# theblackcat102/edgedict

Hardware: AMD Instinct MI355X
Metric: utterances/sec (E6D2, 15 s audio) (higher is better)
Workload: dtype bf16; 1 GPU; E6D2 full training step (dither+log-mel+stack3+SpecAugment masks -> 6x1024 LSTM encoder, 2x time reduction -> 2x256 LSTM prediction net -> joint 640 -> RNN-T loss -> backward -> grad all-reduce -> Adam); 64 x 15 s utterances per GPU, U=64, V=2048, ragged lengths; lattice [64,201,65,2048]; global_batch=64, parallelism=dp1

## Files before the change

edgedict_amd/csrc/encoder_stack.hip:

```cpp
#include <stdio.h>
#include <stdlib.h>

#include <algorithm>
#include <mutex>
#include <vector>

#include "stack_kernels.hpp"

int ed_gemm_quiet_partials(int dtype_in, const void* A, long long lda, int a_kmajor, const void* B,
                           long long ldb, int b_kmajor, int M, int N, int K, int split_k,
                           int max_wg_per_cu, float* partials, int* slices, hipStream_t stream);

namespace {

__device__ __forceinline__ uint4 pack8(const float* v) {
    uint4 o;
    o.x = (unsigned)f32_to_bf16(v[0]) | ((unsigned)f32_to_bf16(v[1]) << 16);
    o.y = (unsigned)f32_to_bf16(v[2]) | ((unsigned)f32_to_bf16(v[3]) << 16);
    o.z = (unsigned)f32_to_bf16(v[4]) | ((unsigned)f32_to_bf16(v[5]) << 16);
    o.w = (unsigned)f32_to_bf16(v[6]) | ((unsigned)f32_to_bf16(v[7]) << 16);
    return o;
}
__device__ __forceinline__ int row_of_kap(int kap, int H) { return ((kap >> 4) & 3) * H + (kap >> 6) * 16 + (kap & 15); }

__global__ void pack_wih_kernel(const float* __restrict__ W, const float* __restrict__ b_ih,
                                const float* __restrict__ b_hh, bf16_t* __restrict__ Wp,
                                bf16_t* __restrict__ Wt, float* __restrict__ bp, int H, int I) {
    const long long n = 4ll * H * I;
    for (long long i = (long long)blockIdx.x * blockDim.x + threadIdx.x; i < n;
         i += (long long)gridDim.x * blockDim.x) {
        const int row = (int)(i / I), k = (int)(i % I);
        const int g = row / H, j = row % H;
        const int kap = ed_gate_col(g, j);
        const bf16_t v = f32_to_bf16(W[i]);
        Wp[(long long)kap * I + k] = v;
        if (Wt) Wt[(long long)k * 4 * H + kap] = v;
        if (k == 0) bp[kap] = b_ih[row] + b_hh[row];
    }
}
__global__ void pack_wih8_kernel(const float* __restrict__ W, const float* __restrict__ b_ih,
                                 const float* __restrict__ b_hh, bf16_t* __restrict__ Wp, float* __restrict__ bp, int H,
                                 int I) {
    const int I8 = I >> 3;
    const long long n8 = 4ll * H * I8;
    for (long long c = (long long)blockIdx.x * blockDim.x + threadIdx.x; c < n8; c += (long long)gridDim.x * blockDim.x) {
        const int kap = (int)(c / I8), k8 = (int)(c % I8);
        const int row = row_of_kap(kap, H);
        float v[8];
        const float4 a = *reinterpret_cast<const float4*>(W + (long long)row * I + k8 * 8);
        const float4 b = *reinterpret_cast<const float4*>(W + (long long)row * I + k8 * 8 + 4);
        v[0] = a.x; v[1] = a.y; v[2] = a.z; v[3] = a.w; v[4] = b.x; v[5] = b.y; v[6] = b.z; v[7] = b.w;
        *reinterpret_cast<uint4*>(Wp + (long long)kap * I + k8 * 8) = pack8(v);
        if (k8 == 0) bp[kap] = b_ih[row] + b_hh[row];
    }
}
__global__ __launch_bounds__(256) void pack_wih_t_kernel(const float* __restrict__ W, bf16_t* __restrict__ Wt, int H,
                                                         int I) {
    __shared__ __attribute__((aligned(16))) bf16_t tile[64][64 + 8];
    const int kt = (I + 63) >> 6;
    const int kap0 = (blockIdx.x / kt) * 64, k0 = (blockIdx.x % kt) * 64;
    const int tid = threadIdx.x;
    for (int q = tid; q < 64 * 16; q += 256) {
        const int r = q >> 4, c4 = (q & 15) * 4;
        const int row = row_of_kap(kap0 + r, H);
        float v[4] = {0.f, 0.f, 0.f, 0.f};
        if ((I & 3) == 0 && k0 + c4 + 3 < I) {
            const float4 a = *reinterpret_cast<const float4*>(W + (long long)row * I + k0 + c4);
            v[0] = a.x; v[1] = a.y; v[2] = a.z; v[3] = a.w;
        } else {
            for (int e = 0; e < 4; ++e)
                if (k0 + c4 + e < I) v[e] = W[(long long)row * I + k0 + c4 + e];
        }
        for (int e = 0; e < 4; ++e) tile[c4 + e][r] = f32_to_bf16(v[e]);
    }
    __syncthreads();
    for (int q = tid; q < 64 * 8; q += 256) {
        const int k = q >> 3, c8 = (q & 7) * 8;
        if (k0 + k < I)
            *reinterpret_cast<uint4*>(Wt + (long long)(k0 + k) * 4 * H + kap0 + c8) = *reinterpret_cast<const uint4*>(&tile[k][c8]);
    }
}
__global__ void pack_whh_fwd_kernel(const float* __restrict__ W, bf16_t* __restrict__ out, int H) {
    const long long n8 = 4ll * H * H / 8;
    const int KS = H >> 5;
    for (long long c = (long long)blockIdx.x * blockDim.x + threadIdx.x; c < n8; c += (long long)gridDim.x * blockDim.x) {
        const int lane = (int)(c & 63);
        const long long blk = c >> 6;
        const int g = (int)(blk & 3), ks = (int)((blk >> 2) % KS), ub = (int)((blk >> 2) / KS);
        const int row = g * H + ub * 16 + (lane & 15);
        const int k = ks * 32 + (lane >> 4) * 8;
        float v[8];
        const float4 a = *reinterpret_cast<const float4*>(W + (long long)row * H + k);
        const float4 b = *reinterpret_cast<const float4*>(W + (long long)row * H + k + 4);
        v[0] = a.x; v[1] = a.y; v[2] = a.z; v[3] = a.w; v[4] = b.x; v[5] = b.y; v[6] = b.z; v[7] = b.w;
        *reinterpret_cast<uint4*>(out + c * 8) = pack8(v);
    }
}
__global__ void pack_whh_bwd_kernel(const float* __restrict__ W, bf16_t* __restrict__ out, int H) {
    const long long n8 = 4ll * H * H / 8;
    const int KS = H >> 3;
    for (long long c = (long long)blockIdx.x * blockDim.x + threadIdx.x; c < n8; c += (long long)gridDim.x * blockDim.x) {
        const int lane = (int)(c & 63);
        const long long blk = c >> 6;
        const int n2 = (int)(blk & 1), ks = (int)((blk >> 1) % KS), nb = (int)((blk >> 1) / KS);
        const int unit = (nb * 2 + n2) * 16 + (lane & 15);
        const int kap = ks * 32 + (lane >> 4) * 8;
        const float* src = W + (long long)row_of_kap(kap, H) * H + unit;
        float v[8];
#pragma unroll
        for (int e = 0; e < 8; ++e) v[e] = src[(long long)e * H];
        *reinterpret_cast<uint4*>(out + c * 8) = pack8(v);
    }
}
__global__ void unpermute_rows_kernel(const float* __restrict__ src, long long slice_stride, int S,
                                      float* __restrict__ dst, float* __restrict__ dst2, int H, int K,
                                      int accumulate) {
    const long long n = 4ll * H * K;
    for (long long i = (long long)blockIdx.x * blockDim.x + threadIdx.x; i < n;
         i += (long long)gridDim.x * blockDim.x) {
        const int row = (int)(i / K), k = (int)(i % K);
        const long long o = (long long)ed_gate_col(row / H, row % H) * K + k;
        float v = 0.f;
        for (int sl = 0; sl < S; ++sl) v += src[sl * slice_stride + o];
        dst[i] = accumulate ? dst[i] + v : v;
        if (dst2) dst2[i] = accumulate ? dst2[i] + v : v;
    }
}

__global__ void unpermute_rows4_kernel(const float* __restrict__ src, long long slice_stride, int S,
                                       float* __restrict__ dst, float* __restrict__ dst2, int H, int K,
                                       int accumulate) {
    const int K4 = K >> 2;
    const long long n4 = 4ll * H * K4;
    for (long long c = (long long)blockIdx.x * blockDim.x + threadIdx.x; c < n4; c += (long long)gridDim.x * blockDim.x) {
        const int row = (int)(c / K4), k = (int)(c % K4) * 4;
        const long long o = (long long)ed_gate_col(row / H, row % H) * K + k;
        float4 v = make_float4(0.f, 0.f, 0.f, 0.f);
        for (int sl = 0; sl < S; ++sl) {
            const float4 p = *reinterpret_cast<const float4*>(src + sl * slice_stride + o);
            v.x += p.x; v.y += p.y; v.z += p.z; v.w += p.w;
        }
        const long long i = (long long)row * K + k;
        if (accumulate) {
            const float4 d = *reinterpret_cast<const float4*>(dst + i);
            *reinterpret_cast<float4*>(dst + i) = make_float4(d.x + v.x, d.y + v.y, d.z + v.z, d.w + v.w);
            if (dst2) {
                const float4 e = *reinterpret_cast<const float4*>(dst2 + i);
                *reinterpret_cast<float4*>(dst2 + i) = make_float4(e.x + v.x, e.y + v.y, e.z + v.z, e.w + v.w);
            }
        } else {
            *reinterpret_cast<float4*>(dst + i) = v;
            if (dst2) *reinterpret_cast<float4*>(dst2 + i) = v;
        }
    }
}
int unpermute_rows(const float* src, long long slice_stride, int S, float* dst, float* dst2, int H, int K, int accumulate,
                   hipStream_t s) {
    const bool vec = K % 4 == 0 && slice_stride % 4 == 0 && (uintptr_t)src % 16 == 0 && (uintptr_t)dst % 16 == 0 &&
                     (uintptr_t)dst2 % 16 == 0;
    if (vec)
        hipLaunchKernelGGL(unpermute_rows4_kernel, dim3(ed_grid_for(4ll * H * K / 4, 256, 4096)), dim3(256), 0, s, src,
                           slice_stride, S, dst, dst2, H, K, accumulate);
    else
        hipLaunchKernelGGL(unpermute_rows_kernel, dim3(ed_grid_for(4ll * H * K, 256, 4096)), dim3(256), 0, s, src,
                           slice_stride, S, dst, dst2, H, K, accumulate);
    ED_CHECK_LAUNCH("unpermute_rows_kernel");
    return ED_OK;
}

struct Runtime {
    std::mutex mu;
    hipStream_t R = nullptr, W = nullptr;
    int prio_hi = 0;
    hipEvent_t tev[2][2] = {{nullptr, nullptr}, {nullptr, nullptr}};
    int tlaunches[2] = {0, 0};
    int tkind[2] = {0, 0}, tsteps[2] = {0, 0};
    bool time_each = false;
    static constexpr int STAMP_SLOTS = 4096;
    unsigned long long* stamps[2] = {nullptr, nullptr};
    int stamp_used[2] = {0, 0};
    unsigned long long* stamp_slot(int i, hipStream_t s) {
        if (!time_each) return nullptr;
        if (!stamps[i] && hipMalloc((void**)&stamps[i], (size_t)STAMP_SLOTS * 16) != hipSuccess) {
            stamps[i] = nullptr;
            return nullptr;
        }
        if (stamp_used[i] == 0) {
            if (hipMemsetAsync(stamps[i], 0, (size_t)STAMP_SLOTS * 16, s) != hipSuccess) return nullptr;
            if (hipMemset2DAsync(stamps[i], 16, 0xff, 8, STAMP_SLOTS, s) != hipSuccess) return nullptr;
        }
        if (stamp_used[i] >= STAMP_SLOTS) return nullptr;
        return stamps[i] + 2 * (size_t)stamp_used[i]++;
    }
    unsigned* wsr_err_host = nullptr;
    unsigned* wsr_err_dev = nullptr;
    hipStream_t lazy(hipStream_t& s) {
        if (!s && hipStreamCreateWithPriority(&s, hipStreamNonBlocking, prio_hi) != hipSuccess) s = nullptr;
        return s;
    }
    hipStream_t S[ED_STACK_MAX_SLOTS] = {};
    std::vector<hipEvent_t> pool;
    size_t used = 0;
    hipEvent_t get() {
        if (used == pool.size()) {
            hipEvent_t e;
            if (hipEventCreateWithFlags(&e, hipEventDisableTiming) != hipSuccess) return nullptr;
            pool.push_back(e);
        }
        return pool[used++];
    }
};
std::mutex g_rt_mu;
std::vector<Runtime*> g_rt;

Runtime* runtime_for_current_device() {
    int dev = 0;
    if (hipGetDevice(&dev) != hipSuccess) return nullptr;
    std::lock_guard<std::mutex> registry(g_rt_mu);
    if ((int)g_rt.size() <= dev) g_rt.resize(dev + 1, nullptr);
    if (!g_rt[dev]) {
        Runtime* r = new Runtime();
        int lo = 0, hi = 0;
        if (hipDeviceGetStreamPriorityRange(&lo, &hi) != hipSuccess) lo = hi = 0;
        const char* e = getenv("EDGEDICT_AUX_PRIORITY");
        const bool aux_high = e && e[0] == '1';
        r->prio_hi = hi;
        bool ok = hipStreamCreateWithPriority(&r->R, hipStreamNonBlocking, hi) == hipSuccess &&
                  hipStreamCreateWithPriority(&r->W, hipStreamNonBlocking, aux_high ? hi : lo) == hipSuccess &&
                  hipStreamCreateWithPriority(&r->S[0], hipStreamNonBlocking, hi) == hipSuccess;
        if (!ok) {
            delete r;
            return nullptr;
        }
        for (int i = 0; i < 2; ++i)
            for (int j = 0; j < 2; ++j)
                if (hipEventCreate(&r->tev[i][j]) != hipSuccess) r->tev[i][j] = nullptr;
        if (hipHostMalloc((void**)&r->wsr_err_host, 64, hipHostMallocMapped) == hipSuccess) {
            r->wsr_err_host[0] = r->wsr_err_host[1] = r->wsr_err_host[2] = 0;
            if (hipHostGetDevicePointer((void**)&r->wsr_err_dev, r->wsr_err_host, 0) != hipSuccess)
                r->wsr_err_dev = nullptr;
        }
        g_rt[dev] = r;
    }
    return g_rt[dev];
}

struct Geom {
    int T, f, m, cf, off, nchunks;
};

size_t align256(size_t x) { return (x + 255) / 256 * 256; }
constexpr int LNB_GRID = 128;
constexpr int LNB_GRID_TOP = 512;

struct WsLayout {
    std::vector<size_t> frag0, frag1, dC, lnpart;
    std::vector<size_t> himg;
    size_t himg_stride = 0;
    std::vector<size_t> gimg;
    size_t gimg_stride = 0;
    std::vector<size_t> skpart;
    size_t tmpW = 0, tmpB = 0, dX0 = 0, wsr_sync = 0, total = 0;
};
constexpr size_t SYNC_FFLAG = 0, SYNC_BFLAG = 8 * 512, SYNC_FCNT = 2 * 8 * 512;
constexpr size_t SYNC_BCNT = SYNC_FCNT + (size_t)8 * LPW_CNT_STRIDE;
constexpr size_t SYNC_GCNT = 16 * 1024;
constexpr size_t WSR_SYNC_BYTES = (SYNC_GCNT + (size_t)8 * SK_CNT_LINES * 64) * 4;
static_assert(SYNC_BCNT + (size_t)8 * LPW_CNT_STRIDE <= SYNC_GCNT, "sync region layout");

WsLayout ws_layout(const edgedict_stack_desc_t* d) {
    WsLayout w;
    const size_t B16 = (size_t)(d->B + 15) / 16 * 16;
    size_t off = 0;
    size_t maxK = d->H;
    for (int l = 0; l < d->L; ++l) {
        const size_t fb = align256(B16 * 4 * d->H * sizeof(bf16_t));
        w.frag0.push_back(off); off += fb;
        w.frag1.push_back(off); off += fb;
        if ((size_t)d->layers[l].I > maxK) maxK = d->layers[l].I;
    }
    for (int l = 0; l < d->L; ++l) {
        w.dC.push_back(off);
        off += align256((size_t)d->B * d->H * sizeof(float));
    }
    {
        int f = 1;
        std::vector<int> fl(d->L);
        for (int l = d->L - 1; l >= 0; --l) { f *= max(1, d->layers[l].reduce); fl[l] = f; }
        for (int l = 0; l < d->L; ++l) {
            const int cf = max(1, d->chunk) * fl[l];
            const int nch = (d->layers[l].T + cf - 1) / cf;
            w.lnpart.push_back(off);
            off += align256((size_t)(nch * LNB_GRID + LNB_GRID_TOP) * 2 * d->H * sizeof(float));
        }
    }
    w.tmpW = off; off += align256((size_t)8 * 4 * d->H * maxK * sizeof(float));
    w.tmpB = off; off += align256((size_t)4 * d->H * sizeof(float));
    w.dX0 = off; off += align256((size_t)d->T0 * d->B * d->I0 * sizeof(bf16_t));
    w.wsr_sync = off; off += WSR_SYNC_BYTES;
    w.himg_stride = align256(B16 * d->H * sizeof(bf16_t));
    for (int l = 0; l < d->L; ++l) {
        w.himg.push_back(off);
        off += (size_t)(d->layers[l].T + 1) * w.himg_stride;
    }
    const bool infer = (d->flags & EDGEDICT_STACK_INFERENCE) != 0;
    w.gimg_stride = align256(B16 * 4 * d->H * sizeof(bf16_t));
    for (int l = 0; l < d->L; ++l) {
        w.gimg.push_back(off);
        if (!infer) off += (size_t)(d->layers[l].T + 1) * w.gimg_stride;
    }
    for (int l = 0; l < d->L; ++l) {
        w.skpart.push_back(off);
        if (!infer) off += align256((size_t)2 * (d->H / 64 + 1) * 4 * 64 * 64 * sizeof(float));
    }
    w.total = off;
    return w;
}

int validate(const edgedict_stack_desc_t* d, std::vector<Geom>& g, bool backward) {
    ED_CHECK_ARG(d && d->layers, "encoder_stack: null descriptor");
    ED_CHECK_ARG(d->L >= 1 && d->L <= ED_STACK_MAX_SLOTS, "encoder_stack: 1..%d layers supported (got %d)", ED_STACK_MAX_SLOTS, d->L);
    ED_CHECK_ARG(d->B >= 1 && d->H >= 32 && d->H % 32 == 0 && d->H <= 2048, "encoder_stack: need B >= 1, H %% 32 == 0, H <= 2048 (B=%d H=%d)", d->B, d->H);
    ED_CHECK_ARG(d->chunk >= 1, "encoder_stack: chunk must be >= 1");
    ED_CHECK_ARG(d->T0 >= 1 && d->I0 >= 8 && d->I0 % 8 == 0 && d->I0 <= 1024, "encoder_stack: bad input geometry (T0=%d I0=%d)", d->T0, d->I0);
    ED_CHECK_ARG(d->x && d->in_gamma && d->in_beta && d->in_mean && d->in_rstd && d->out && d->ws, "encoder_stack: null pointer in descriptor");
    g.resize(d->L);
    int f = 1;
    for (int l = d->L - 1; l >= 0; --l) {
        const edgedict_stack_layer_t& y = d->layers[l];
        ED_CHECK_ARG(y.reduce == 1 || y.reduce == 2, "encoder_stack: layer %d: time reduction must be 1 or 2", l);
        f *= y.reduce;
        g[l].f = f;
        g[l].T = y.T;
    }
    int T = d->T0, I = d->I0;
    for (int l = 0; l < d->L; ++l) {
        const edgedict_stack_layer_t& y = d->layers[l];
        ED_CHECK_ARG(y.T == T && y.I == I, "encoder_stack: layer %d geometry (T=%d I=%d) does not follow from the layers above (T=%d I=%d)", l, y.T, y.I, T, I);
        ED_CHECK_ARG(!y.residual || y.I == d->H, "encoder_stack: layer %d: residual needs I == H", l);
        ED_CHECK_ARG(y.drop_p >= 0.f && y.drop_p < 1.f, "encoder_stack: layer %d: dropout probability must be in [0, 1)", l);
        ED_CHECK_ARG(y.wih_p && y.bias_p && y.whh_f && y.ln_gamma && y.ln_beta && y.X && y.G && y.Yx && y.Cx && y.mean && y.rstd, "encoder_stack: layer %d: null pointer", l);
        if (backward)
            ED_CHECK_ARG(y.whh_b && y.dZ && (l == 0 || y.dX) && y.dW_ih && y.dW_hh && y.db && y.dgamma && y.dbeta, "encoder_stack: layer %d: null backward pointer", l);
        g[l].m = g[0].f / g[l].f;
        g[l].cf = d->chunk * g[l].f;
        g[l].nchunks = (y.T + g[l].cf - 1) / g[l].cf;
        T = (T + y.reduce - 1) / y.reduce;
        I = d->H;
    }
    ED_CHECK_ARG(d->ws_bytes >= ws_layout(d).total, "encoder_stack: workspace too small");
    return ED_OK;
}

struct Pace {
    static bool allows(int w, int l, int m_l, int m_min_running) {
        const int period = max(1, m_l / max(1, m_min_running));
        return period <= 1 || ((w + period * 1024 - (l % period)) % period) == 0;
    }
};

int margin_launches(const edgedict_stack_desc_t* d, const std::vector<Geom>& g, bool backward) {
    const int P = d->chunk * g[0].f;
    if (d->lag > 0) return max(1, d->lag - P + (backward ? 1 : 0));
    static const int mf = [] { const char* e = getenv("EDGEDICT_STACK_MARGIN_F"); return e ? atoi(e) : 0; }();
    static const int mb = [] { const char* e = getenv("EDGEDICT_STACK_MARGIN_B"); return e ? atoi(e) : 0; }();
    if (backward ? mb > 0 : mf > 0) return backward ? mb : mf;
    return backward ? 6 : 3;
}

#define ED_TRY(expr)            \
    do {                        \
        int st__ = (expr);      \
        if (st__ != ED_OK) return st__; \
    } while (0)

struct ScheduleTrace {
    int32_t* step_launch = nullptr;
    int32_t* chunk_enqueued = nullptr;
    std::vector<int> toff, coff;
    int launches = 0, max_slots = 0;
};
thread_local ScheduleTrace* g_trace = nullptr;
#define ED_DEV(expr)                      \
    do {                                  \
        if (!g_trace) ED_TRY(expr);       \
    } while (0)

struct Streams {
    hipStream_t C, R, R2, W;
    int split;
    int which(int l) const { return l >= split ? 1 : 0; }
    hipStream_t RS(int l) const { return which(l) ? R2 : R; }
    hipStream_t S[ED_STACK_MAX_SLOTS];
    bool serial;
    Runtime* rt;
    std::unique_lock<std::mutex> lock;
    hipEvent_t shared_ev = nullptr;
    hipStream_t shared_src = nullptr;
    int share(hipStream_t src) {
        if (serial) return ED_OK;
        shared_ev = rt->get();
        ED_CHECK_ARG(shared_ev != nullptr, "encoder_stack: event creation failed");
        ED_CHECK_HIP(hipEventRecord(shared_ev, src));
        shared_src = src;
        return ED_OK;
    }
    void unshare() { shared_ev = nullptr; shared_src = nullptr; }
    int chain(hipStream_t src, hipStream_t waiter) {
        if (serial || src == waiter) return ED_OK;
        if (shared_ev && src == shared_src) {
            ED_CHECK_HIP(hipStreamWaitEvent(waiter, shared_ev, 0));
            return ED_OK;
        }
        hipEvent_t e = rt->get();
        ED_CHECK_ARG(e != nullptr, "encoder_stack: event creation failed");
        ED_CHECK_HIP(hipEventRecord(e, src));
        ED_CHECK_HIP(hipStreamWaitEvent(waiter, e, 0));
        return ED_OK;
    }
    int record(hipEvent_t& e, hipStream_t src) {
        if (serial) return ED_OK;
        e = rt->get();
        ED_CHECK_ARG(e != nullptr, "encoder_stack: event creation failed");
        ED_CHECK_HIP(hipEventRecord(e, src));
        return ED_OK;
    }
    int wait(hipStream_t waiter, hipEvent_t e) {
        if (serial || !e) return ED_OK;
        ED_CHECK_HIP(hipStreamWaitEvent(waiter, e, 0));
        return ED_OK;
    }
};

int open_streams(const edgedict_stack_desc_t* d, void* stream_, Streams& st) {
    st.C = (hipStream_t)stream_;
    st.serial = (d->flags & EDGEDICT_STACK_SERIAL) != 0 || g_trace != nullptr;
    st.rt = nullptr;
    if (st.serial) {
        st.R = st.R2 = st.W = st.C;
        for (auto& x : st.S) x = st.C;
        return ED_OK;
    }
    st.rt = runtime_for_current_device();
    ED_CHECK_ARG(st.rt != nullptr, "encoder_stack: could not create the internal streams");
    st.lock = std::unique_lock<std::mutex>(st.rt->mu);
    st.rt->used = 0;
    st.R = st.rt->R;
    st.R2 = st.rt->R;
    for (int i = 0; i < ED_STACK_MAX_SLOTS; ++i) {
        st.S[i] = st.rt->S[0];
        if ((d->flags & EDGEDICT_STACK_SIDE_STREAM_PER_LAYER) && i > 0) {
// ... 220 lines not shown
            sl.nsteps = t1 - t;
            sl.layer = l;
            ran[Lc.nslot].l = l;
            ran[Lc.nslot].t0 = t;
            ran[Lc.nslot].t1 = t1;
            ++Lc.nslot;
            next_t[l] = t1;
            if (g_trace)
                for (int tt = t; tt < t1; ++tt) g_trace->step_launch[g_trace->toff[l] + tt] = g_trace->launches;
        }
        if (Lc.nslot == 0) {
            ED_CHECK_ARG(++idle < 4096, "encoder_stack: forward schedule made no progress");
            continue;
        }
        idle = 0;
        ++launches;
        Lc.stamp = st.rt ? st.rt->stamp_slot(0, st.R) : nullptr;
        Lc.err = gerr;
        Lc.trace = g_wsr_trace;
        ED_DEV(ed_stack_launch_fwd_lpw(Lc, st.R));
        if (g_trace) {
            g_trace->max_slots = max(g_trace->max_slots, Lc.nslot);
            ++g_trace->launches;
        }
        for (int pass = 0; pass < 2; ++pass) {
            hipStream_t S = pass == 0 ? st.S[0] : st.C;
            EdChunkNorm items[ED_STACK_MAX_SLOTS];
            int idx[ED_STACK_MAX_SLOTS], ni = 0;
            for (int i = 0; i < Lc.nslot; ++i) {
                const int l = ran[i].l;
                if (side(l) != S) continue;
                const edgedict_stack_layer_t& y = d->layers[l];
                EdChunkNorm& e = items[ni];
                e.Yx1 = bptr(y.Yx) + BH;
                e.X = y.residual ? bptr(y.X) : nullptr;
                e.gamma = y.ln_gamma;
                e.beta = y.ln_beta;
                if (l + 1 < L) {
                    e.out = bptr(d->layers[l + 1].X);
                    e.out_st = BH;
                    e.out_sb = H;
                } else {
                    e.out = bptr(d->out);
                    e.out_st = H;
                    e.out_sb = (long long)T_out * H;
                }
                e.mean = y.mean;
                e.rstd = y.rstd;
                e.T = y.T;
                e.t0 = ran[i].t0;
                e.t1 = ran[i].t1;
                e.reduce = y.reduce;
                const DropCfg dc = drop_of(y);
                e.drop_thresh = dc.thresh; e.drop_seed = dc.seed; e.drop_scale = dc.scale; e.drop_T = dc.T_out;
                idx[ni++] = i;
            }
            if (ni == 0) continue;
            if (soft) {
                const unsigned* cp[ED_STACK_MAX_SLOTS];
                unsigned tg[ED_STACK_MAX_SLOTS];
                for (int j = 0; j < ni; ++j) {
                    cp[j] = cnt + (size_t)ran[idx[j]].l * LPW_CNT_STRIDE;
                    tg[j] = (unsigned)WGS * (unsigned)ran[idx[j]].t1;
                }
                ED_DEV(ed_stack_wait_counters(cp, tg, ni, gerr, S));
            } else {
                ED_TRY(st.chain(st.R, S));
            }
            ED_DEV(ed_stack_multi_norm(items, ni, B, H, d->eps, S));
            for (int j = 0; j < ni; ++j) {
                const int i = idx[j];
                const int l = ran[i].l, k = ran[i].t0 / g[l].cf;
                if (l + 1 >= L || ran[i].t1 != min(g[l].T, (k + 1) * g[l].cf)) continue;
                ED_DEV(input_gemm(d, g, l + 1, k, S));
                if (g_trace) g_trace->chunk_enqueued[g_trace->coff[l + 1] + k] = g_trace->launches;
                if (soft) ED_DEV(ed_stack_set_flag(fflag + (l + 1) * 512 + k, S));
                else ED_TRY(st.record(Eg[l + 1][k], S));
                queued[l + 1][k] = 1;
                ready_w[l + 1][k] = w + margin;
            }
            if (st.serial) break;
        }
    }
    if (st.rt && st.rt->tev[0][1]) {
        ED_CHECK_HIP(hipEventRecord(st.rt->tev[0][1], st.R));
        st.rt->tlaunches[0] = launches;
    }
    ED_TRY(st.chain(st.R, st.C));
    for (int l = 0; l < L; ++l) ED_TRY(st.chain(st.S[l], st.C));
    return ED_OK;
}

int lpw_steps(const edgedict_stack_desc_t* d) {
    const char* e_on = getenv("EDGEDICT_STACK_LPW");
    const char* e_n = getenv("EDGEDICT_LPW_STEPS");
    const int on = e_on ? atoi(e_on) : 1, want = e_n ? atoi(e_n) : min(d->chunk, 16);
    if (!on || !ed_stack_lpw_supported(d->B, d->H)) return 0;
    {
        const size_t B16 = (size_t)(d->B + 15) / 16 * 16;
        const size_t stride = align256(B16 * d->H * sizeof(bf16_t));
        for (int l = 0; l < d->L; ++l)
            if ((size_t)(d->layers[l].T + 1) * stride >= (1ull << 32)) return 0;
        if (!g_trace && device_cus() < (d->H >> 4) * ((d->B + 63) >> 6)) return 0;
    }
    bool reduces = false;
    for (int l = 0; l < d->L; ++l) reduces = reduces || d->layers[l].reduce == 2;
    int ns = max(1, min(want, d->chunk));
    while (ns > 1 && (d->chunk % ns != 0 || (reduces && (ns & 1)))) --ns;
    if (reduces && (ns & 1)) return 0;
    return ns;
}

int sk_bwd_steps(const edgedict_stack_desc_t* d) {
    const char* e_on = getenv("EDGEDICT_STACK_BWD_SK");
    const char* e_n = getenv("EDGEDICT_SK_STEPS");
    const int on = e_on ? atoi(e_on) : 1, want = e_n ? atoi(e_n) : min(d->chunk, 16);
    if (!on || !ed_stack_sk_supported(d->B, d->H)) return 0;
    for (int l = 0; l < d->L; ++l)
        if (!d->layers[l].whh_s) return 0;
    {
        const size_t B16 = (size_t)(d->B + 15) / 16 * 16;
        const size_t stride = align256(B16 * 4 * d->H * sizeof(bf16_t));
        for (int l = 0; l < d->L; ++l)
            if ((size_t)(d->layers[l].T + 1) * stride >= (1ull << 32)) return 0;
        if (!g_trace && 2 * device_cus() < (d->H >> 6) * 4) return 0;
    }
    int ns = max(1, min(want, d->chunk));
    while (ns > 1 && d->chunk % ns != 0) --ns;
    return ns;
}

}

extern "C" int edgedict_stack_forward(const edgedict_stack_desc_t* d, void* stream_) {
    std::vector<Geom> g;
    ED_TRY(validate(d, g, false));
    const int B = d->B, H = d->H, L = d->L;
    const long long BH = (long long)B * H;
    const WsLayout wl = ws_layout(d);
    char* ws = (char*)d->ws;
    Streams st;
    ED_TRY(open_streams(d, stream_, st));
    static const int fwd_r2 = [] { const char* e = getenv("EDGEDICT_STACK_FWD_R2"); return e ? atoi(e) : 1; }();
    if (fwd_r2 && !st.serial && st.R2 == st.R) st.R2 = st.C;
    st.split = L;
    if (st.R2 != st.R) {
        st.split = L / 2;
        for (int l = 0; l < L; ++l)
            if (d->layers[l].reduce == 2) { st.split = l + 1; break; }
        if (st.split >= L) st.split = L / 2;
    }

    ED_DEV(ed_stack_input_norm(d->x_dtype, d->x, d->in_gamma, d->in_beta, bptr(d->layers[0].X),
                               d->in_mean, d->in_rstd, B, d->T0, d->I0, d->eps, st.C));
    const int lpw_ns = lpw_steps(d);
    if (lpw_ns && (poison_on() || lpw_data_poll()))
        ED_DEV(ed_stack_fill(ws + wl.himg[0], 0xff,
                             wl.himg[L - 1] + (size_t)(d->layers[L - 1].T + 1) * wl.himg_stride - wl.himg[0], st.C));
    if (st.rt) {
        st.rt->tkind[0] = lpw_ns ? 1 : 0;
        st.rt->tsteps[0] = lpw_ns;
    }
    for (int l0 = 0; l0 < L; l0 += 8) {
        EdInitStates A;
        A.n = min(8, L - l0);
        A.B = B;
        A.H = H;
        for (int j = 0; j < A.n; ++j) {
            const int l = l0 + j;
            const edgedict_stack_layer_t& y = d->layers[l];
            A.h0[j] = d->h0 ? d->h0 + l * BH : nullptr;
            A.c0[j] = d->c0 ? d->c0 + l * BH : nullptr;
            A.Yx0[j] = bptr(y.Yx);
            A.Cx0[j] = y.Cx;
            A.hfrag[j] = bptr(ws + (lpw_ns ? wl.himg[l] : wl.frag0[l]));
        }
        ED_DEV(ed_stack_init_states(A, st.C));
    }
    if (lpw_ns) ED_DEV(ed_stack_zero(ws + wl.wsr_sync, SYNC_BCNT * sizeof(unsigned), st.C));
    ED_TRY(st.chain(st.C, st.R));
    if (st.R2 != st.R) ED_TRY(st.chain(st.C, st.R2));
    for (int l = 0; l < L; ++l) ED_TRY(st.chain(st.C, st.S[l]));

    static const int soft_env = [] { const char* e = getenv("EDGEDICT_STACK_SOFT_WAIT"); return e ? atoi(e) : 1; }();
    const bool soft = soft_env && !st.serial && L <= 8;
    if (lpw_ns) return forward_lpw(d, g, st, wl, lpw_ns, soft);
    unsigned* fflag = reinterpret_cast<unsigned*>(ws + wl.wsr_sync) + SYNC_FFLAG;
    unsigned* gerr = (st.rt && st.rt->wsr_err_dev) ? st.rt->wsr_err_dev + 2 : nullptr;
    if (soft) {
        for (int l = 0; l < L; ++l) ED_CHECK_ARG(g[l].nchunks <= 512, "encoder_stack: too many chunks for the flag table");
        ED_DEV(ed_stack_zero(fflag, (size_t)8 * 512 * sizeof(unsigned), st.C));
        ED_TRY(st.chain(st.C, st.R));
        if (st.R2 != st.R) ED_TRY(st.chain(st.C, st.R2));
        for (int l = 0; l < L; ++l) ED_TRY(st.chain(st.C, st.S[l]));
    }
    std::vector<std::vector<hipEvent_t>> Eg(L);
    std::vector<std::vector<char>> queued(L);
    for (int l = 0; l < L; ++l) {
        Eg[l].assign(g[l].nchunks, nullptr);
        queued[l].assign(g[l].nchunks, 0);
    }
    int next_g0 = 0;
    auto feed_layer0 = [&](int upto) -> int {
        for (; next_g0 < g[0].nchunks && next_g0 <= upto; ++next_g0) {
            ED_DEV(input_gemm(d, g, 0, next_g0, st.S[0]));
            if (g_trace) g_trace->chunk_enqueued[g_trace->coff[0] + next_g0] = g_trace->launches;
            if (soft) ED_DEV(ed_stack_set_flag(fflag + next_g0, st.S[0]));
            else ED_TRY(st.record(Eg[0][next_g0], st.S[0]));
            queued[0][next_g0] = 1;
        }
        return ED_OK;
    };
    ED_TRY(feed_layer0(1));

    const int margin = margin_launches(d, g, false);
    std::vector<int> next_t(L, 0), stepped_w(L, -2);
    std::vector<std::vector<int>> ready_w(L);
    for (int l = 0; l < L; ++l) ready_w[l].assign(g[l].nchunks, l == 0 ? 0 : 0x3fffffff);
    int launches = 0, idle = 0;
    if (st.rt) st.rt->stamp_used[0] = 0;
    if (st.rt && st.rt->tev[0][0]) ED_CHECK_HIP(hipEventRecord(st.rt->tev[0][0], st.R));
    const int T_out = (g[L - 1].T + d->layers[L - 1].reduce - 1) / d->layers[L - 1].reduce;
    struct Done { int l, k; };
    for (int w = 0;; ++w) {
        bool finished = true;
        for (int l = 0; l < L; ++l) finished = finished && next_t[l] >= g[l].T && stepped_w[l] < w - 1;
        if (finished) break;
        EdFwdLaunch Lcs[2];
        for (auto& x : Lcs) {
            x.nstep = x.nnorm = 0;
            x.B = B; x.H = H; x.eps = d->eps;
        }
        Done done[ED_STACK_MAX_SLOTS];
        int ndone = 0;
        for (int l = 0; l < L; ++l) {
            const edgedict_stack_layer_t& y = d->layers[l];
            EdFwdLaunch& Lc = Lcs[st.which(l)];
            if (stepped_w[l] == w - 1) {
                const int t = next_t[l] - 1;
                int ta = -1, tb = -1;
                if (y.reduce == 1) ta = t;
                else if (t & 1) { ta = t - 1; tb = t; }
                else if (t == g[l].T - 1) ta = t;
                if (ta >= 0) {
                    const int tau = ta / y.reduce;
                    EdFwdNorm& n = Lc.norm[Lc.nnorm++];
                    n.y0 = bptr(y.Yx) + (long long)(ta + 1) * BH;
                    n.r0 = y.residual ? bptr(y.X) + (long long)ta * BH : nullptr;
                    n.y1 = tb >= 0 ? bptr(y.Yx) + (long long)(tb + 1) * BH : nullptr;
                    n.r1 = (tb >= 0 && y.residual) ? bptr(y.X) + (long long)tb * BH : nullptr;
                    n.gamma = y.ln_gamma;
                    n.beta = y.ln_beta;
                    if (l + 1 < L) {
                        n.out = bptr(d->layers[l + 1].X) + (long long)tau * BH;
                        n.out_stride = H;
                    } else {
                        n.out = bptr(d->out) + (long long)tau * H;
                        n.out_stride = (long long)T_out * H;
                    }
                    n.mean0 = y.mean + (long long)ta * B;
                    n.rstd0 = y.rstd + (long long)ta * B;
                    n.mean1 = tb >= 0 ? y.mean + (long long)tb * B : nullptr;
                    n.rstd1 = tb >= 0 ? y.rstd + (long long)tb * B : nullptr;
                    n.scale = y.reduce == 1 ? 1.f : 0.5f;
                    const DropCfg dc = drop_of(y);
                    n.drop_thresh = dc.thresh; n.drop_seed = dc.seed; n.drop_scale = dc.scale; n.drop_T = dc.T_out;
                    n.tau = tau;
                }
                const int k = t / g[l].cf;
                if (l + 1 < L && t == min(g[l].T, (k + 1) * g[l].cf) - 1) {
                    done[ndone].l = l;
                    done[ndone].k = k;
                    ++ndone;
                }
            }
            const int t = next_t[l];
            if (t >= g[l].T) continue;
            const int k = t / g[l].cf;
            const bool opens = (t % g[l].cf == 0);
            if (opens && !(queued[l][k] && w >= ready_w[l][k]) && l > 0) continue;
            int m_min = g[l].m;
            for (int j = 0; j < l; ++j)
                if (next_t[j] < g[j].T) m_min = min(m_min, g[j].m);
            if (!Pace::allows(w, l, g[l].m, m_min)) continue;
            if (opens) {
                if (l == 0) ED_TRY(feed_layer0(k + 2));
                ED_CHECK_ARG(queued[l][k], "encoder_stack: schedule violated (layer %d chunk %d)", l, k);
                if (!soft) ED_TRY(st.wait(st.RS(l), Eg[l][k]));
            }
            EdFwdStep& sl = Lc.step[Lc.nstep++];
            sl.wait_flag = (soft && opens) ? fflag + l * 512 + k : nullptr;
            bf16_t* f0 = bptr(ws + wl.frag0[l]);
            bf16_t* f1 = bptr(ws + wl.frag1[l]);
            sl.G_t = bptr(y.G) + (long long)t * B * 4 * H;
            sl.hfrag_in = (t & 1) ? f1 : f0;
            sl.hfrag_out = (t & 1) ? f0 : f1;
            sl.Y_t = bptr(y.Yx) + (long long)(t + 1) * BH;
            sl.C_prev = y.Cx + (long long)t * BH;
            sl.C_t = y.Cx + (long long)(t + 1) * BH;
            sl.Wfrag = bptr(y.whh_f);
            stepped_w[l] = w;
            next_t[l] = t + 1;
            if (g_trace) g_trace->step_launch[g_trace->toff[l] + t] = g_trace->launches;
        }
        if (Lcs[0].nstep + Lcs[0].nnorm + Lcs[1].nstep + Lcs[1].nnorm == 0) {
            ED_CHECK_ARG(++idle < 4096, "encoder_stack: forward schedule made no progress");
            continue;
// ... 21 lines not shown
        }
    }
    const int Wtot = launches;
    if (st.rt && st.rt->tev[0][1]) {
        ED_CHECK_HIP(hipEventRecord(st.rt->tev[0][1], st.R));
        st.rt->tlaunches[0] = Wtot;
    }
    ED_TRY(st.chain(st.R, st.C));
    if (st.R2 != st.R) ED_TRY(st.chain(st.R2, st.C));
    for (int l = 0; l < L; ++l) ED_TRY(st.chain(st.S[l], st.C));
    return ED_OK;
}

extern "C" int edgedict_stack_pack_sk(const float* w_hh, int H, void* whh_s, void* stream_) {
    ED_CHECK_ARG(H >= 64 && H % 64 == 0 && H <= 1024, "stack_pack_sk: needs H %% 64 == 0 and H <= 1024 (got %d)", H);
    ED_CHECK_ARG(w_hh && whh_s, "stack_pack_sk: null pointer");
    return ed_stack_pack_sk(w_hh, (bf16_t*)whh_s, H, (hipStream_t)stream_);
}

extern "C" int edgedict_stack_wsr_set_trace(void* device_buffer) {
    g_wsr_trace = (long long*)device_buffer;
    return ED_OK;
}

extern "C" int edgedict_stack_wsr_error(void) {
    Runtime* r = runtime_for_current_device();
    std::unique_lock<std::mutex> lock;
    if (r) lock = std::unique_lock<std::mutex>(r->mu);
    if (!r || !r->wsr_err_host) return 0;
    volatile unsigned* p = r->wsr_err_host;
    if (!(p[0] | p[1] | p[2])) return 0;
    (void)hipDeviceSynchronize();
    const unsigned code = p[2] ? p[2] : (p[1] ? p[1] : p[0]);
    p[0] = 0;
    p[1] = 0;
    p[2] = 0;
    return (int)code;
}

extern "C" void* edgedict_stack_error_words(int host) {
    Runtime* r = runtime_for_current_device();
    std::unique_lock<std::mutex> lock;
    if (r) lock = std::unique_lock<std::mutex>(r->mu);
    if (!r || !r->wsr_err_host || !r->wsr_err_dev) {
        ed_set_error("stack_error_words: no device runtime");
        return nullptr;
    }
    return host ? (void*)r->wsr_err_host : (void*)r->wsr_err_dev;
}

extern "C" int edgedict_stack_schedule(const edgedict_stack_desc_t* d, int backward, int32_t* step_launch,
                                       int32_t* chunk_enqueued, int32_t* n_launches, int32_t* max_slots) {
    ED_CHECK_ARG(d && step_launch && chunk_enqueued && n_launches && max_slots, "stack_schedule: null pointer");
    ScheduleTrace tr;
    {
        std::vector<Geom> g;
        ED_TRY(validate(d, g, backward != 0));
        int to = 0, co = 0;
        for (int l = 0; l < d->L; ++l) {
            tr.toff.push_back(to);
            tr.coff.push_back(co);
            to += g[l].T;
            co += g[l].nchunks;
        }
        for (int i = 0; i < to; ++i) step_launch[i] = -1;
        for (int i = 0; i < co; ++i) chunk_enqueued[i] = -1;
    }
    tr.step_launch = step_launch;
    tr.chunk_enqueued = chunk_enqueued;
    g_trace = &tr;
    const int rc = backward ? edgedict_stack_backward(d, nullptr) : edgedict_stack_forward(d, nullptr);
    g_trace = nullptr;
    *n_launches = tr.launches;
    *max_slots = tr.max_slots;
    return rc;
}

extern "C" int edgedict_stack_last_timing(int backward, float* ms, int* launches) {
    ED_CHECK_ARG(ms && launches, "stack_last_timing: null pointer");
    Runtime* r = runtime_for_current_device();
    std::unique_lock<std::mutex> lock;
    if (r) lock = std::unique_lock<std::mutex>(r->mu);
    const int i = backward ? 1 : 0;
    ED_CHECK_ARG(r && r->tev[i][0] && r->tev[i][1] && r->tlaunches[i] > 0, "stack_last_timing: nothing recorded");
    ED_CHECK_HIP(hipEventSynchronize(r->tev[i][1]));
    ED_CHECK_HIP(hipEventElapsedTime(ms, r->tev[i][0], r->tev[i][1]));
    *launches = r->tlaunches[i];
    return ED_OK;
}

extern "C" int edgedict_stack_last_mode(int backward, int* kind, int* steps_per_launch) {
    ED_CHECK_ARG(kind && steps_per_launch, "stack_last_mode: null pointer");
    Runtime* r = runtime_for_current_device();
    std::unique_lock<std::mutex> lock;
    if (r) lock = std::unique_lock<std::mutex>(r->mu);
    ED_CHECK_ARG(r, "stack_last_mode: no device runtime");
    *kind = r->tkind[backward ? 1 : 0];
    *steps_per_launch = r->tsteps[backward ? 1 : 0];
    return ED_OK;
}

extern "C" int edgedict_stack_time_launches(int on) {
    Runtime* r = runtime_for_current_device();
    std::unique_lock<std::mutex> lock;
    if (r) lock = std::unique_lock<std::mutex>(r->mu);
    ED_CHECK_ARG(r, "stack_time_launches: no device runtime");
    r->time_each = on != 0;
    return ED_OK;
}

extern "C" int edgedict_stack_launch_times(int backward, float* sum_ms, int* launches) {
    ED_CHECK_ARG(sum_ms && launches, "stack_launch_times: null pointer");
    Runtime* r = runtime_for_current_device();
    std::unique_lock<std::mutex> lock;
    if (r) lock = std::unique_lock<std::mutex>(r->mu);
    const int i = backward ? 1 : 0;
    ED_CHECK_ARG(r && r->stamps[i] && r->stamp_used[i] > 0,
                 "stack_launch_times: nothing recorded (edgedict_stack_time_launches(1) first)");
    const int n = r->stamp_used[i];
    std::vector<unsigned long long> h(2 * (size_t)n);
    ED_CHECK_HIP(hipStreamSynchronize(r->R));
    ED_CHECK_HIP(hipMemcpy(h.data(), r->stamps[i], h.size() * sizeof(unsigned long long), hipMemcpyDeviceToHost));
    double ticks = 0.0;
    int ok = 0;
    for (int k = 0; k < n; ++k)
        if (h[2 * k + 1] > h[2 * k]) {
            ticks += (double)(h[2 * k + 1] - h[2 * k]);
            ++ok;
        }
    ED_CHECK_ARG(ok > 0, "stack_launch_times: no launch stamped");
    *sum_ms = (float)(ticks * 1e-5);
    *launches = ok;
    return ED_OK;
}

extern "C" int edgedict_stack_launch_stamps(int backward, unsigned long long* out, int max_launches, int* launches) {
    ED_CHECK_ARG(out && launches && max_launches > 0, "stack_launch_stamps: bad arguments");
    Runtime* r = runtime_for_current_device();
    std::unique_lock<std::mutex> lock;
    if (r) lock = std::unique_lock<std::mutex>(r->mu);
    const int i = backward ? 1 : 0;
    ED_CHECK_ARG(r && r->stamps[i] && r->stamp_used[i] > 0,
                 "stack_launch_stamps: nothing recorded (edgedict_stack_time_launches(1) first)");
    const int n = min(max_launches, r->stamp_used[i]);
    ED_CHECK_HIP(hipDeviceSynchronize());
    ED_CHECK_HIP(hipMemcpy(out, r->stamps[i], (size_t)n * 16, hipMemcpyDeviceToHost));
    *launches = n;
    return ED_OK;
}

extern "C" int edgedict_stack_backward(const edgedict_stack_desc_t* d, void* stream_) {
    std::vector<Geom> g;
    ED_TRY(validate(d, g, true));
    ED_CHECK_ARG(d->dout && d->d_in_gamma && d->d_in_beta, "encoder_stack: null backward pointer in descriptor");
    ED_CHECK_ARG(!(d->flags & EDGEDICT_STACK_INFERENCE), "encoder_stack: backward on a descriptor flagged EDGEDICT_STACK_INFERENCE");
    const int B = d->B, H = d->H, L = d->L;
    const long long BH = (long long)B * H;
    const WsLayout wl = ws_layout(d);
    char* ws = (char*)d->ws;
    Streams st;
    ED_TRY(open_streams(d, stream_, st));
    st.R2 = st.R;
    st.split = L;
    const int T_out = (g[L - 1].T + d->layers[L - 1].reduce - 1) / d->layers[L - 1].reduce;

    static const int soft_env = [] { const char* e = getenv("EDGEDICT_STACK_SOFT_WAIT"); return e ? atoi(e) : 1; }();
    const bool soft = soft_env && !st.serial && L <= 8;
    unsigned* bflag = reinterpret_cast<unsigned*>(ws + wl.wsr_sync) + SYNC_BFLAG;
    unsigned* gerr = (st.rt && st.rt->wsr_err_dev) ? st.rt->wsr_err_dev + 2 : nullptr;
    if (soft)
        for (int l = 0; l < L; ++l) ED_CHECK_ARG(g[l].nchunks <= 512, "encoder_stack: too many chunks for the flag table");
    const int sk_ns = sk_bwd_steps(d);
    if (st.rt) {
        st.rt->tkind[1] = sk_ns ? 2 : 0;
        st.rt->tsteps[1] = sk_ns;
    }
    unsigned* cntb = reinterpret_cast<unsigned*>(ws + wl.wsr_sync) + SYNC_BCNT;
    unsigned* gcnt = reinterpret_cast<unsigned*>(ws + wl.wsr_sync) + SYNC_GCNT;
    if (sk_ns) {
        if (poison_on())
            for (int l = 0; l < L; ++l) {
                ED_DEV(ed_stack_fill(ws + wl.gimg[l], 0xff, (size_t)(d->layers[l].T + 1) * wl.gimg_stride, st.C));
                ED_DEV(ed_stack_fill(ws + wl.skpart[l], 0xff, (size_t)2 * (H / 64) * 4 * 64 * 64 * sizeof(float), st.C));
            }
    }
    if (soft || sk_ns)
        ED_DEV(ed_stack_zero(ws + wl.wsr_sync + SYNC_BFLAG * sizeof(unsigned), WSR_SYNC_BYTES - SYNC_BFLAG * sizeof(unsigned), st.C));
    ED_DEV(ed_stack_zero(ws + wl.dC[0], wl.dC[L - 1] + (size_t)BH * sizeof(float) - wl.dC[0], st.C));
    ED_TRY(st.chain(st.C, st.R));
    if (st.R2 != st.R) ED_TRY(st.chain(st.C, st.R2));
    for (int l = 0; l < L; ++l) ED_TRY(st.chain(st.C, st.S[l]));
    ED_TRY(st.chain(st.C, st.W));

    std::vector<std::vector<hipEvent_t>> Eb(L);
    std::vector<std::vector<char>> queued(L);
    for (int l = 0; l < L; ++l) {
        Eb[l].assign(g[l].nchunks, nullptr);
        queued[l].assign(g[l].nchunks, l == L - 1 ? 1 : 0);
    }
    {
        const edgedict_stack_layer_t& y = d->layers[L - 1];
        hipStream_t S = st.S[L - 1];
        const DropCfg dcT = drop_of(y);
        for (int k = g[L - 1].nchunks - 1; k >= 0; --k) {
            const int t0 = k * g[L - 1].cf, t1 = min(y.T, t0 + g[L - 1].cf);
            ED_DEV(ed_stack_ln_bwd(bptr(d->dout), H, (long long)T_out * H, bptr(y.Yx) + BH,
                                   y.residual ? bptr(y.X) : nullptr, y.ln_gamma, y.mean, y.rstd, bptr(y.dZ),
                                   (float*)(ws + wl.lnpart[L - 1]) + (size_t)k * LNB_GRID * 2 * H, LNB_GRID, B, H,
                                   t0, t1, y.reduce, S, dcT.thresh, dcT.seed, dcT.scale, dcT.T_out));
            if (soft) ED_DEV(ed_stack_set_flag(bflag + (L - 1) * 512 + k, S));
            else ED_TRY(st.record(Eb[L - 1][k], S));
        }
    }
    std::vector<int> deferred;

    const int acc_grads = (d->flags & EDGEDICT_STACK_ACCUM_GRADS) ? 1 : 0;
    auto weight_grads = [&](int l, int t0, int t1, bool first, bool last_of_all) -> int {
        if (g_trace) {
            if (t0 == 0 && d->grads_final) d->grads_final(l, d->grads_final_user);
            return ED_OK;
        }
        const edgedict_stack_layer_t& y = d->layers[l];
        const int M = (t1 - t0) * B;
        const long long r0 = (long long)t0 * B;
        float* tmpW = (float*)(ws + wl.tmpW);
        float* tmpB = (float*)(ws + wl.tmpB);
        const int sk = d->split_k > 0 ? d->split_k : (last_of_all ? 8 : 2);
        const int cap = last_of_all ? 4 : 2;
        const int acc = (acc_grads || !first) ? 1 : 0;
        int S = 1;
        ED_TRY(ed_gemm_quiet_partials(ED_BF16, bptr(y.G) + r0 * 4 * H, 4ll * H, 0, bptr(y.X) + r0 * y.I, y.I, 0,
                                      4 * H, y.I, M, sk, cap, tmpW, &S, st.W));
        ED_TRY(unpermute_rows(tmpW, 4ll * H * y.I, S, y.dW_ih, nullptr, H, y.I, acc, st.W));
        ED_TRY(ed_gemm_quiet_partials(ED_BF16, bptr(y.G) + r0 * 4 * H, 4ll * H, 0, bptr(y.Yx) + r0 * H, H, 0,
                                      4 * H, H, M, sk, cap, tmpW, &S, st.W));
        ED_TRY(unpermute_rows(tmpW, 4ll * H * H, S, y.dW_hh, nullptr, H, H, acc, st.W));
        ED_TRY(ed_stack_zero(tmpB, (size_t)4 * H * sizeof(float), st.W));
        ED_TRY(edgedict_colsum(ED_BF16, bptr(y.G) + r0 * 4 * H, 4ll * H, tmpB, M, 4 * H, st.W));
        hipLaunchKernelGGL(unpermute_rows_kernel, dim3(ed_grid_for(4ll * H, 256, 4096)), dim3(256),
                           0, st.W, tmpB, 0, 1, y.db, y.db_hh, H, 1, acc);
        ED_CHECK_LAUNCH("unpermute_rows_kernel");
        if (t0 == 0 && d->grads_final) d->grads_final(l, d->grads_final_user);
        return ED_OK;
    };
    int dw_seg = 1 << 20;
    if (const char* e = getenv("EDGEDICT_STACK_DW_SEG")) dw_seg = max(1, atoi(e));
    if (d->flags & EDGEDICT_STACK_DW_AT_END) dw_seg = 1 << 20;
    int tail_split = 0;
    if (const char* e = getenv("EDGEDICT_STACK_TAIL_SPLIT")) tail_split = atoi(e);

    int margin = margin_launches(d, g, true);
    std::vector<int> next_t(L, 0);
    std::vector<std::vector<int>> ready_w(L);
    for (int l = 0; l < L; ++l) ready_w[l].assign(g[l].nchunks, l == L - 1 ? 0 : 0x3fffffff);
    auto after_recurrence = [&](int l, hipStream_t waiter) -> int { return st.chain(st.RS(l), waiter); };
    auto chunk_done = [&](int l, int k, int w) -> int {
            const edgedict_stack_layer_t& y = d->layers[l];
            if (l > 0) {
                const edgedict_stack_layer_t& z = d->layers[l - 1];
                const int t0 = k * g[l].cf, t1 = min(y.T, t0 + g[l].cf);
                const long long r0 = (long long)t0 * B;
                hipStream_t S = st.S[l];
                ED_TRY(after_recurrence(l, S));
                ED_DEV(edgedict_gemm(ED_BF16, ED_BF16, bptr(y.G) + r0 * 4 * H, 4ll * H, 1,
                                     y.wih_t ? y.wih_t : y.wih_p, y.wih_t ? 4ll * H : y.I,
                                     y.wih_t ? 1 : 0, bptr(y.dX) + r0 * y.I, y.I, (t1 - t0) * B, y.I,
                                     4 * H, nullptr, nullptr, y.dX == y.dZ ? 1 : 0, 1, S));
                const int u0 = k * g[l - 1].cf, u1 = min(z.T, u0 + g[l - 1].cf);
                ED_DEV(ed_stack_ln_bwd(bptr(y.dX), (long long)B * y.I, y.I, bptr(z.Yx) + BH,
                                       z.residual ? bptr(z.X) : nullptr, z.ln_gamma, z.mean, z.rstd,
                                       bptr(z.dZ), (float*)(ws + wl.lnpart[l - 1]) + (size_t)k * LNB_GRID * 2 * H,
                                       LNB_GRID, B, H, u0, u1, z.reduce, S, drop_of(z).thresh, drop_of(z).seed,
                                       drop_of(z).scale, drop_of(z).T_out));
                if (soft) ED_DEV(ed_stack_set_flag(bflag + (l - 1) * 512 + k, S));
                else ED_TRY(st.record(Eb[l - 1][k], S));
                queued[l - 1][k] = 1;
                ready_w[l - 1][k] = w + margin;
                if (g_trace) g_trace->chunk_enqueued[g_trace->coff[l - 1] + k] = g_trace->launches;
            }
            const int k_split = (l <= 1 && tail_split > 1 && g[l].nchunks >= 2 * tail_split && dw_seg >= g[l].nchunks &&
                                 !(d->flags & EDGEDICT_STACK_DW_AT_END))
                                    ? g[l].nchunks / tail_split : 0;
            if (k_split > 0 && k == k_split) {
                ED_TRY(after_recurrence(l, st.W));
                ED_TRY(weight_grads(l, k * g[l].cf, y.T, true, false));
            } else if (k_split > 0 && k == 0) {
                ED_TRY(after_recurrence(l, st.W));
                ED_TRY(weight_grads(l, 0, k_split * g[l].cf, false, l == 0));
            } else if (k_split == 0 && k % dw_seg == 0) {
                if (d->flags & EDGEDICT_STACK_DW_AT_END) {
                    if (k == 0) deferred.push_back(l);
                } else {
                    const int k1 = min(g[l].nchunks, k + dw_seg);
                    const int t0 = k * g[l].cf, t1 = min(y.T, k1 * g[l].cf);
                    ED_TRY(after_recurrence(l, st.W));
                    ED_TRY(weight_grads(l, t0, t1, k1 == g[l].nchunks, l == 0 && k == 0));
                }
            }
        return ED_OK;
    };
    int launches = 0, idle = 0;
    if (st.rt) st.rt->stamp_used[1] = 0;
    if (st.rt && st.rt->tev[1][0]) ED_CHECK_HIP(hipEventRecord(st.rt->tev[1][0], st.R));
    struct Done { int l, k, t; };
    if (sk_ns) {
        const int WGS = (H >> 6) * 4;
        const int n_cu = ed_device_cus();
        const int max_slots = max(1, min(ED_STACK_MAX_SLOTS, (g_trace ? 256 : n_cu) / WGS));
        const char* e_m = getenv("EDGEDICT_LPW_MARGIN_B");
        margin = (e_m && atoi(e_m) > 0) ? atoi(e_m) : 2;
        for (int w = 0;; ++w) {
            bool finished = true;
            for (int l = 0; l < L; ++l) finished = finished && next_t[l] >= g[l].T;
            if (finished) break;
            EdSkLaunch Ls;
            Ls.nslot = 0;
            Ls.B = B;
            Ls.H = H;
            Ls.trace = g_wsr_trace;
            Done done[ED_STACK_MAX_SLOTS];
            int ndone = 0;
            int order[ED_STACK_MAX_SLOTS];
            for (int l = 0; l < L; ++l) order[l] = l;
            std::stable_sort(order, order + L, [&](int a, int b) { return g[a].T - next_t[a] > g[b].T - next_t[b]; });
            for (int oi = 0; oi < L; ++oi) {
                const int l = order[oi];
                const edgedict_stack_layer_t& y = d->layers[l];
                if (next_t[l] >= g[l].T || Ls.nslot >= max_slots) continue;
                const int t = g[l].T - 1 - next_t[l];
                const int k = t / g[l].cf;
                const bool opens = (t == min(g[l].T, (k + 1) * g[l].cf) - 1);
                if (opens && !(queued[l][k] && w >= ready_w[l][k])) continue;
                int m_min = g[l].m;
                for (int j = 0; j < l; ++j)
                    if (next_t[j] > 0 && next_t[j] < g[j].T) m_min = min(m_min, g[j].m);
                if (!Pace::allows(w, l, g[l].m, m_min)) continue;
                if (opens && !soft) ED_TRY(st.wait(st.R, Eb[l][k]));
                int t_end = max(k * g[l].cf, t - sk_ns + 1);
                if (t_end - k * g[l].cf == 1) t_end = k * g[l].cf;
                EdSkSlot& ss = Ls.slot[Ls.nslot++];
                ss.G = bptr(y.G) + (long long)t * B * 4 * H;
                ss.img = bptr(ws + wl.gimg[l]);
                ss.img_stride = (long long)wl.gimg_stride;
                ss.img_bytes = (long long)(y.T + 1) * (long long)wl.gimg_stride;
                ss.dY = bptr(y.dZ) + (long long)t * BH;
                ss.Cx = y.Cx;
                ss.dC = (float*)(ws + wl.dC[l]);
                ss.Wsk = bptr(y.whh_s);
                ss.part = (float*)(ws + wl.skpart[l]);
                ss.counter = cntb + (size_t)l * LPW_CNT_STRIDE;
                ss.gcounter = gcnt + (size_t)l * SK_CNT_LINES * 64;
                ss.done = (unsigned)next_t[l];
                ss.wait_flag = (soft && opens) ? bflag + l * 512 + k : nullptr;
                ss.t0 = t;
                ss.nsteps = t - t_end + 1;
                ss.T = y.T;
                ss.layer = l;
                if (t_end == k * g[l].cf) {
                    done[ndone].l = l; done[ndone].k = k; done[ndone].t = t_end;
                    ++ndone;
                }
                next_t[l] += t - t_end + 1;
                if (g_trace)
                    for (int tt = t_end; tt <= t; ++tt) g_trace->step_launch[g_trace->toff[l] + tt] = g_trace->launches;
            }
            if (Ls.nslot == 0) {
                ED_CHECK_ARG(++idle < 4096, "encoder_stack: backward schedule made no progress");
                continue;
            }
            idle = 0;
            ++launches;
            Ls.stamp = st.rt ? st.rt->stamp_slot(1, st.R) : nullptr;
            Ls.err = gerr;
            ED_DEV(ed_stack_launch_bwd_sk(Ls, st.R));
            if (g_trace) {
                g_trace->max_slots = max(g_trace->max_slots, Ls.nslot);
                ++g_trace->launches;
            }
            if (ndone > 1) ED_TRY(st.share(st.R));
            for (int i = 0; i < ndone; ++i) ED_TRY(chunk_done(done[i].l, done[i].k, w));
            st.unshare();
        }
    } else
    for (int w = 0;; ++w) {
        bool finished = true;
        for (int l = 0; l < L; ++l) finished = finished && next_t[l] >= g[l].T;
        if (finished) break;
        EdBwdLaunch Lcs[2];
        for (auto& x : Lcs) {
            x.nstep = 0;
            x.B = B; x.H = H;
        }
        Done done[ED_STACK_MAX_SLOTS];
        int ndone = 0;
        for (int l = L - 1; l >= 0; --l) {
            const edgedict_stack_layer_t& y = d->layers[l];
            if (next_t[l] >= g[l].T) continue;
            const int t = g[l].T - 1 - next_t[l];
            const int k = t / g[l].cf;
            const bool opens = (t == min(g[l].T, (k + 1) * g[l].cf) - 1);
            if (opens && !(queued[l][k] && w >= ready_w[l][k])) continue;
            int m_min = g[l].m;
            for (int j = 0; j < l; ++j)
                if (next_t[j] > 0 && next_t[j] < g[j].T) m_min = min(m_min, g[j].m);
            if (!Pace::allows(w, l, g[l].m, m_min)) continue;
            if (opens && !soft) ED_TRY(st.wait(st.RS(l), Eb[l][k]));
            EdBwdLaunch& Lc = Lcs[st.which(l)];
            EdBwdStep& sl = Lc.step[Lc.nstep++];
            sl.wait_flag = (soft && opens) ? bflag + l * 512 + k : nullptr;
            bf16_t* f0 = bptr(ws + wl.frag0[l]);
            bf16_t* f1 = bptr(ws + wl.frag1[l]);
            sl.G_t = bptr(y.G) + (long long)t * B * 4 * H;
            sl.gfrag_in = (t == g[l].T - 1) ? nullptr : (((t + 1) & 1) ? f1 : f0);
            sl.gfrag_out = (t == 0) ? nullptr : ((t & 1) ? f1 : f0);
            sl.dY_t = bptr(y.dZ) + (long long)t * BH;
            sl.C_t = y.Cx + (long long)(t + 1) * BH;
            sl.C_prev = y.Cx + (long long)t * BH;
            sl.dC = (float*)(ws + wl.dC[l]);
            sl.WTfrag = bptr(y.whh_b);
            if (t == k * g[l].cf) {
                done[ndone].l = l; done[ndone].k = k; done[ndone].t = t;
                ++ndone;
            }
            ++next_t[l];
            if (g_trace) g_trace->step_launch[g_trace->toff[l] + t] = g_trace->launches;
        }
        if (Lcs[0].nstep + Lcs[1].nstep == 0) {
            ED_CHECK_ARG(++idle < 4096, "encoder_stack: backward schedule made no progress");
            continue;
        }
        idle = 0;
        ++launches;
        Lcs[0].stamp = st.rt ? st.rt->stamp_slot(1, st.R) : nullptr;
        Lcs[1].stamp = nullptr;
        Lcs[0].err = Lcs[1].err = gerr;
        ED_DEV(ed_stack_launch_bwd(Lcs[0], st.R));
        if (st.R2 != st.R) ED_DEV(ed_stack_launch_bwd(Lcs[1], st.R2));
        if (g_trace) {
            g_trace->max_slots = max(g_trace->max_slots, Lcs[0].nstep + Lcs[1].nstep);
            ++g_trace->launches;
        }
        for (int i = 0; i < ndone; ++i) ED_TRY(chunk_done(done[i].l, done[i].k, w));
    }
    const int Wtot = launches;
    if (st.rt && st.rt->tev[1][1]) {
        ED_CHECK_HIP(hipEventRecord(st.rt->tev[1][1], st.R));
        st.rt->tlaunches[1] = Wtot;
    }
    {
        const edgedict_stack_layer_t& y = d->layers[0];
        bf16_t* dX0 = bptr(ws + wl.dX0);
        ED_TRY(st.chain(st.RS(0), st.S[0]));
        ED_DEV(edgedict_gemm(ED_BF16, ED_BF16, y.G, 4ll * H, 1, y.wih_t ? y.wih_t : y.wih_p,
                             y.wih_t ? 4ll * H : y.I, y.wih_t ? 1 : 0, dX0, y.I, y.T * B, y.I, 4 * H,
                             nullptr, nullptr, 0, 1, st.S[0]));
        ED_DEV(ed_stack_input_norm_bwd(d->x_dtype, d->x, dX0, d->in_mean, d->in_rstd, d->d_in_gamma,
                                       d->d_in_beta, B, d->T0, d->I0, st.S[0]));
        for (int l = 1; l < L; ++l) ED_TRY(st.chain(st.S[l], st.S[0]));
        for (int l = 0; l < L; ++l) {
            const edgedict_stack_layer_t& z = d->layers[l];
            const float* part = (const float*)(ws + wl.lnpart[l]);
            ED_DEV(ed_stack_sum_parts(part, g[l].nchunks * LNB_GRID, H, z.dgamma, z.dbeta, st.S[0]));
        }
    }
    if (!deferred.empty()) {
        ED_TRY(st.chain(st.R, st.W));
        if (st.R2 != st.R) ED_TRY(st.chain(st.R2, st.W));
        for (int l : deferred) ED_TRY(weight_grads(l, 0, d->layers[l].T, true, false));
    }
    ED_TRY(st.chain(st.R, st.C));
    if (st.R2 != st.R) ED_TRY(st.chain(st.R2, st.C));
    for (int l = 0; l < L; ++l) ED_TRY(st.chain(st.S[l], st.C));
    ED_TRY(st.chain(st.W, st.C));
    return ED_OK;
}
```

edgedict_amd/csrc/gemm.hip:

```cpp
#include "common.hpp"
#include "gemm_plan.hpp"
#include "blaslt.hpp"

namespace {

typedef __attribute__((ext_vector_type(8))) __bf16 bf16x8_t;
typedef __attribute__((ext_vector_type(4))) float f32x4_t;

constexpr int BM = 128, BN = 128;
constexpr int THREADS = 256;

template <typename TI> struct Cfg;
template <> struct Cfg<bf16_t> {
    static constexpr int BK = 64;
    static constexpr int ROW = BK + 8;
    static constexpr int VEC = 8;
};
template <> struct Cfg<float> {
    static constexpr int BK = 16;
    static constexpr int ROW = BK + 4;
    static constexpr int VEC = 4;
};

struct GemmArgs {
// ... 256 lines not shown
                    for (int r = 0; r < 4; ++r)
                        sC[(wm * 64 + i * 16 + (lane >> 4) * 4 + r) * CROW + cl] =
                            f32_to_bf16(acc[i][j][r] + bias);
            }
            __syncthreads();
#pragma unroll
            for (int it = 0; it < BM * BN / 8 / THREADS; ++it) {
                const int c = threadIdx.x + it * THREADS;
                const int rl = c / (BN / 8), ch = c % (BN / 8);
                const int row = m0 + rl, col = n0 + ch * 8;
                if (row >= g.M || col >= g.N) continue;
                uint4 v = *reinterpret_cast<const uint4*>(sC + rl * CROW + ch * 8);
                bf16_t* dst = reinterpret_cast<bf16_t*>(C) + (long long)row * g.ldc + col;
                if (g.accumulate) {
                    float x[8], y[8];
                    ElemIO<bf16_t>::load_vec(dst, x);
                    ElemIO<bf16_t>::load_vec(reinterpret_cast<const bf16_t*>(&v), y);
#pragma unroll
                    for (int e = 0; e < 8; ++e) x[e] += y[e];
                    ElemIO<bf16_t>::store_vec(dst, x);
                } else {
                    *reinterpret_cast<uint4*>(dst) = v;
                }
            }
            __syncthreads();
            continue;
        }
    }
#pragma unroll
    for (int j = 0; j < 4; ++j) {
        const int col = n0 + wn * 64 + j * 16 + (lane & 15);
        if (col >= g.N) continue;
        float bias = 0.f;
        if (first_split) {
            if (g.bias1) bias += g.bias1[col];
            if (g.bias2) bias += g.bias2[col];
        }
#pragma unroll
        for (int i = 0; i < 4; ++i) {
#pragma unroll
            for (int r = 0; r < 4; ++r) {
                const int row = m0 + wm * 64 + i * 16 + (lane >> 4) * 4 + r;
                if (row >= g.M) continue;
                const float v = acc[i][j][r] + bias;
                TO* dst = C + (long long)row * g.ldc + col;
                if constexpr (sizeof(TO) == 4) {
                    if (g.partials) g.partials[slice * g.partial_stride + (long long)row * g.N + col] = v;
                    else if (g.split_k > 1) atomicAdd(reinterpret_cast<float*>(dst), v);
                    else if (g.accumulate) *dst = *dst + v;
                    else *dst = v;
                } else {
                    if (g.accumulate) ElemIO<TO>::store(dst, ElemIO<TO>::load(dst) + v);
                    else ElemIO<TO>::store(dst, v);
                }
            }
        }
    }
  }
}

template <typename TI, typename TO, bool FAST>
int launch2(const GemmArgs& g, int a_km, int b_km, dim3 grid, hipStream_t s, int pad) {
    if (a_km && b_km) hipLaunchKernelGGL((gemm_kernel<TI, TO, true, true, FAST>), grid, dim3(THREADS), pad, s, g);
    else if (a_km && !b_km) hipLaunchKernelGGL((gemm_kernel<TI, TO, true, false, FAST>), grid, dim3(THREADS), pad, s, g);
    else if (!a_km && b_km) hipLaunchKernelGGL((gemm_kernel<TI, TO, false, true, FAST>), grid, dim3(THREADS), pad, s, g);
    else hipLaunchKernelGGL((gemm_kernel<TI, TO, false, false, FAST>), grid, dim3(THREADS), pad, s, g);
    ED_CHECK_LAUNCH("gemm");
    return ED_OK;
}
__global__ void reduce_partials_kernel(const float* __restrict__ part, long long stride, int S,
                                       float* __restrict__ C, long long ldc, long long M, int N,
                                       int accumulate) {
    const long long n = M * N;
    for (long long i = (long long)blockIdx.x * blockDim.x + threadIdx.x; i < n;
         i += (long long)gridDim.x * blockDim.x) {
        float a = 0.f;
        for (int s = 0; s < S; ++s) a += part[s * stride + i];
        float* dst = C + (i / N) * ldc + (i % N);
        *dst = accumulate ? *dst + a : a;
    }
}

__global__ void zero_f32(float* p, long long rows, long long cols, long long ld) {
    const long long n = rows * cols;
    for (long long i = (long long)blockIdx.x * blockDim.x + threadIdx.x; i < n;
         i += (long long)gridDim.x * blockDim.x)
        p[(i / cols) * ld + (i % cols)] = 0.f;
}

}

static int pow2_slices(int split_k) {
    int p2 = 1;
    while (p2 < split_k && p2 < 8) p2 *= 2;
    return p2;
}
static bool vec16(const void* p, long long ld, int vec) { return (uintptr_t)p % 16 == 0 && ld % vec == 0; }
static bool nt_ok(const GemmCall& c) {
    if ((uintptr_t)c.bias1 % 16 != 0 || (uintptr_t)c.bias2 % 16 != 0) return false;
    return c.dtype_in == ED_BF16 && c.dtype_out == ED_BF16 && c.a_kmajor && c.b_kmajor && c.split_k == 1 && c.M > 0 &&
           c.N > 0 && c.K >= 64 && c.K % 64 == 0 && c.lda % 8 == 0 && c.ldb % 8 == 0 && c.ldc % 8 == 0 && c.N % 8 == 0 &&
           (uintptr_t)c.A % 16 == 0 && (uintptr_t)c.B % 16 == 0 && (uintptr_t)c.C % 16 == 0;
}
static bool nt256_shape_ok(int M, int N, int K) { return M > 0 && N > 0 && K >= 128 && K % 64 == 0; }
static bool tn256_ok(const GemmCall& c) {
    return ed_env_once("EDGEDICT_GEMM_TN256", 1) && c.M >= 8 && c.N >= 8 && c.K >= 1 && c.M % 8 == 0 && c.N % 8 == 0 &&
           c.lda % 8 == 0 && c.ldb % 8 == 0 && (uintptr_t)c.A % 16 == 0 && (uintptr_t)c.B % 16 == 0;
}

int ed_gemm_plan(const GemmCall& c, GemmPlan& p) {
    p = GemmPlan{};
    const int M = c.M, N = c.N, K = c.K, n_cu = ed_device_cus();
    if (M == 0 || N == 0) return ED_OK;
    p.split = 1;
    const bool has_bias = c.bias1 || c.bias2;
    const bool nt = ed_env_once("EDGEDICT_GEMM_NT", 1) && c.max_wg_per_cu == 0 && nt_ok(c);
    const long long tiles256 = (long long)((M + 255) / 256) * ((N + 255) / 256);
    if (c.lse_part || (nt && ed_env_once("EDGEDICT_GEMM_NT256", 1) && !c.accumulate && nt256_shape_ok(M, N, K) &&
                       tiles256 >= 512)) {
        ED_CHECK_ARG(tiles256 < (1ll << 31), "gemm: too many tiles");
        const int n_tiles = (N + 255) / 256, cus = n_cu - n_cu % 8;
        const int grid = (int)(tiles256 < cus ? tiles256 : cus);
        const bool ring = ed_env_now("EDGEDICT_GEMM_NT256R", 1) &&
                          !(has_bias && tiles256 > grid && ((grid / 8) % n_tiles != 0 || grid % 8 != 0));
        p.kernel = !ring ? ED_K_NT256 : c.lse_part ? ED_K_NT256R_LSE : ED_K_NT256R;
        p.grid = ring ? grid : (unsigned)tiles256;
        p.block = 512;
        p.lds = ring ? ED_NT256R_LDS_BYTES : ED_NT256_LDS_BYTES;
        return ED_OK;
    }
    const bool plain_nt = c.dtype_in == ED_BF16 && c.dtype_out == ED_BF16 && c.a_kmajor && c.b_kmajor && c.split_k == 1 &&
                          c.max_wg_per_cu == 0 && c.lda % 8 == 0 && c.ldb % 8 == 0 && c.ldc % 8 == 0;
    if (plain_nt && !c.accumulate && !c.bias2 && K >= 1 && K <= 1024 && N >= 1024 && (long long)M * N >= (1ll << 28))
        p.vendor = ED_VENDOR_NT_LOGITS;
    else if (plain_nt && !has_bias && K >= 2048 && M <= 4096 && N <= 2048 && M >= 256 &&
             ed_env_once("EDGEDICT_BLASLT_SMALL", 1))
        p.vendor = ED_VENDOR_NT_SMALL;
    if (nt) {
        const int force = ed_env_once("EDGEDICT_GEMM_NT_TILE", 0);
        int tm = 128, tn = 128;
        if (force == 64 || (!force && (long long)((M + 127) / 128) * ((N + 127) / 128) <= 128)) tm = tn = 64;
        else if (force == 256) tm = 256;
        const long long tiles = (long long)((M + tm - 1) / tm) * ((N + tn - 1) / tn);
        ED_CHECK_ARG(tiles < (1ll << 31), "gemm: too many tiles");
        p.kernel = tm == 256 ? ED_K_NT_256X128 : tm == 128 ? ED_K_NT_128 :
                   ed_env_once("EDGEDICT_GEMM_NT_RING", 1) && K >= 1024 && !ed_env_once("EDGEDICT_GEMM_NT_DEBUG", 0)
                       ? ED_K_NT_RING64 : ED_K_NT_64;
        p.grid = (unsigned)tiles;
        p.block = tm == 256 ? 512 : 256;
        return ED_OK;
    }
    const bool dw = c.dtype_in == ED_BF16 && c.dtype_out == ED_F32 && !c.a_kmajor && !c.b_kmajor &&
                    (long long)M * N >= (1ll << 18);
    if (dw && c.partials && K >= 1024 && tn256_ok(c)) {
        const long long tiles = (long long)((M + 255) / 256) * ((N + 127) / 128);
        long long s = n_cu / tiles < c.slice_cap ? n_cu / tiles : c.slice_cap;
        while (s > 1 && s * 8 > (K + 31) / 32) --s;
        if (s < 1) s = 1;
        ED_CHECK_ARG(tiles * s < (1ll << 30), "gemm_tn256: too many tiles");
        const int items = (int)(tiles * s);
        int grid = n_cu < items ? n_cu : items;
        if (grid > 8) grid = grid / 8 * 8;
        const int per = (items + grid - 1) / grid;
        p.kernel = ED_K_TN256;
        p.grid = (items + per - 1) / per;
        p.block = 512;
        p.lds = ED_TN256_LDS_BYTES;
        p.split = (int)s;
        p.k_per_split = (int)(((K + s - 1) / s + 63) / 64 * 64);
        p.reduce_after = !c.unreduced;
        return ED_OK;
    }
    if (dw && (c.max_wg_per_cu > 0 || c.partials) && !has_bias && K >= 4096 && c.lda % 8 == 0 && c.ldb % 8 == 0 &&
        c.ldc % 4 == 0)
        p.vendor = ED_VENDOR_TN_F32;
    const bool f32 = c.dtype_in == ED_F32;
    const int bk = f32 ? 16 : 64, vec = f32 ? 4 : 8, ktiles = (K + bk - 1) / bk;
    int split = c.split_k;
    if (c.partials) split = pow2_slices(split);
    else if (split > 1) split = (split + 7) / 8 * 8;
    if (split > ktiles) split = ktiles > 0 ? ktiles : 1;
    p.split = split;
    p.k_per_split = ktiles > 0 ? ((ktiles + split - 1) / split) * bk : bk;
    p.zero_first = split > 1 && !c.accumulate && !c.partials;
    p.reduce_after = c.partials && !c.unreduced;
    const long long tiles = (long long)((M + BM - 1) / BM) * ((N + BN - 1) / BN);
    ED_CHECK_ARG(tiles < (1ll << 31), "gemm: too many tiles");
    ED_CHECK_ARG(tiles * split < (1ll << 31), "gemm: too many workgroups");
    long long nwg = tiles * split;
    if (c.max_wg_per_cu > 0) {
        long long cap = (long long)c.max_wg_per_cu * n_cu;
        if (split > 1) cap = cap / split * split;
        if (cap >= split && nwg > cap) nwg = cap;
        const int stat = (BM + BN) * (f32 ? Cfg<float>::ROW * 4 : Cfg<bf16_t>::ROW * 2);
        const int want = (160 * 1024) / (c.max_wg_per_cu + 1) + 1024;
        if (want > stat) p.lds = (want - stat + 255) / 256 * 256;
    }
    p.grid = (unsigned)nwg;
    p.block = THREADS;
    const bool fast = vec16(c.A, c.lda, vec) && vec16(c.B, c.ldb, vec) && (c.a_kmajor ? K : M) % vec == 0 &&
                      (c.b_kmajor ? K : N) % vec == 0;
    p.kernel = (f32 ? ED_K_GENERIC_F32_F32 : c.dtype_out == ED_F32 ? ED_K_GENERIC_BF16_F32 : ED_K_GENERIC_BF16_BF16) + fast;
    return ED_OK;
}

static int generic_launch(const GemmCall& c, const GemmPlan& p, hipStream_t s) {
    const int vec = c.dtype_in == ED_F32 ? 4 : 8;
    GemmArgs g;
    g.A = c.A; g.B = c.B; g.C = c.C; g.bias1 = c.bias1; g.bias2 = c.bias2;
    g.lda = c.lda; g.ldb = c.ldb; g.ldc = c.ldc; g.M = c.M; g.N = c.N; g.K = c.K;
    g.a_vec = vec16(c.A, c.lda, vec);
    g.b_vec = vec16(c.B, c.ldb, vec);
    g.c_vec = c.dtype_out == ED_BF16 && vec16(c.C, c.ldc, 8) && c.N % 8 == 0;
    g.accumulate = c.accumulate;
    g.split_k = p.split;
    g.k_per_split = p.k_per_split;
    g.items = (int)((long long)((c.M + BM - 1) / BM) * ((c.N + BN - 1) / BN) * p.split);
    g.partials = c.partials;
    g.partial_stride = (long long)c.M * c.N;
    const dim3 grid(p.grid, 1, 1);
    switch (p.kernel) {
    case ED_K_GENERIC_BF16_BF16_FAST: return launch2<bf16_t, bf16_t, true>(g, c.a_kmajor, c.b_kmajor, grid, s, p.lds);
    case ED_K_GENERIC_BF16_BF16: return launch2<bf16_t, bf16_t, false>(g, c.a_kmajor, c.b_kmajor, grid, s, p.lds);
    case ED_K_GENERIC_BF16_F32_FAST: return launch2<bf16_t, float, true>(g, c.a_kmajor, c.b_kmajor, grid, s, p.lds);
    case ED_K_GENERIC_BF16_F32: return launch2<bf16_t, float, false>(g, c.a_kmajor, c.b_kmajor, grid, s, p.lds);
    case ED_K_GENERIC_F32_F32_FAST: return launch2<float, float, true>(g, c.a_kmajor, c.b_kmajor, grid, s, p.lds);
    default: return launch2<float, float, false>(g, c.a_kmajor, c.b_kmajor, grid, s, p.lds);
    }
}

int ed_gemm_run(const GemmCall& c, const GemmPlan& p, hipStream_t s, int* slices) {
    if (slices) *slices = p.split;
    if (p.kernel == ED_K_NONE) return ED_OK;
    if (p.vendor == ED_VENDOR_TN_F32
            ? ed_blaslt_tn_f32(c.A, c.lda, c.B, c.ldb, (float*)c.C, c.ldc, c.M, c.N, c.K, c.accumulate, s)
            : p.vendor && ed_blaslt_nt_bf16(c.A, c.lda, c.B, c.ldb, c.C, c.ldc, c.M, c.N, c.K, c.bias1, c.accumulate, s)) {
        if (slices) *slices = 1;
        return ED_OK;
    }
    if (p.zero_first) {
        hipLaunchKernelGGL(zero_f32, dim3(ed_grid_for((long long)c.M * c.N, 256)), dim3(256), 0, s, (float*)c.C,
                           (long long)c.M, (long long)c.N, c.ldc);
        ED_CHECK_LAUNCH("gemm zero");
    }
    const int rc = p.kernel == ED_K_TN256 ? ed_gemm_tn256_launch(c, p, s)
                 : p.kernel >= ED_K_NT256R ? ed_gemm_nt256r_launch(c, p, s)
                 : p.kernel == ED_K_NT256 ? ed_gemm_nt256_launch(c, p, s)
                 : p.kernel >= ED_K_NT_64 ? ed_gemm_nt_launch(c, p, s) : generic_launch(c, p, s);
    if (rc != ED_OK || !p.reduce_after) return rc;
    hipLaunchKernelGGL(reduce_partials_kernel, dim3(ed_grid_for((long long)c.M * c.N, 256, 2048)), dim3(256), 0, s,
                       c.partials, (long long)c.M * c.N, p.split, (float*)c.C, c.ldc, (long long)c.M, c.N, c.accumulate);
    ED_CHECK_LAUNCH("gemm reduce_partials");
    return ED_OK;
}

static int gemm_validate(const GemmCall& c, bool bg) {
    if (c.lse_part) {
        ED_CHECK_ARG(nt256_shape_ok(c.M, c.N, c.K) && nt_ok(c),
                     "gemm_nt_lse: needs bf16 K-contiguous operands, K %% 64 == 0, K >= 128, N %% 8 == 0, "
                     "16-byte aligned pointers and leading dimensions (M=%d N=%d K=%d)", c.M, c.N, c.K);
        return ED_OK;
    }
    ED_CHECK_ARG(!bg || (c.max_wg_per_cu >= 1 && c.max_wg_per_cu <= 8), "gemm_bg: max_wg_per_cu must be 1..8");
    ED_CHECK_ARG(!c.partials || c.dtype_out == ED_F32, "gemm_bg: the quiet (partials) form needs an fp32 output");
    ED_CHECK_ARG(!c.partials || (!c.bias1 && !c.bias2), "gemm_bg: the quiet (partials) form takes no bias");
    ED_CHECK_ARG(c.dtype_in == ED_F32 || c.dtype_in == ED_BF16, "gemm: bad input dtype %d", c.dtype_in);
    ED_CHECK_ARG(c.dtype_out == ED_F32 || c.dtype_out == ED_BF16, "gemm: bad output dtype %d", c.dtype_out);
    ED_CHECK_ARG(!(c.dtype_in == ED_F32 && c.dtype_out == ED_BF16), "gemm: fp32 inputs with bf16 output is not supported");
    ED_CHECK_ARG(c.M >= 0 && c.N >= 0 && c.K >= 0, "gemm: negative dimension");
    ED_CHECK_ARG(c.split_k >= 1, "gemm: split_k must be >= 1");
    ED_CHECK_ARG(c.split_k == 1 || c.dtype_out == ED_F32, "gemm: split_k > 1 needs an fp32 output (atomic +=)");
    ED_CHECK_ARG(c.M == 0 || c.N == 0 || (c.C && (c.K == 0 || (c.A && c.B))), "gemm: null operand");
    return ED_OK;
}
static int gemm_go(const GemmCall& c, bool bg, void* stream, int* slices = nullptr) {
    GemmPlan p;
    int rc = gemm_validate(c, bg);
    if (rc == ED_OK) rc = ed_gemm_plan(c, p);
    return rc == ED_OK ? ed_gemm_run(c, p, (hipStream_t)stream, slices) : rc;
}

int ed_gemm_quiet_partials(int dtype_in, const void* A, long long lda, int a_kmajor, const void* B,
                           long long ldb, int b_kmajor, int M, int N, int K, int split_k,
                           int max_wg_per_cu, float* partials, int* slices, hipStream_t stream) {
    ED_CHECK_ARG(partials, "gemm: quiet product without a partials buffer");
    return gemm_go({dtype_in, ED_F32, A, lda, a_kmajor, B, ldb, b_kmajor, partials, N, M, N, K, nullptr, nullptr, 0, split_k,
                    max_wg_per_cu, partials, 8, true, nullptr}, false, stream, slices);
}

extern "C" int edgedict_gemm(int dtype_in, int dtype_out, const void* A, long long lda, int a_kmajor,
                             const void* B, long long ldb, int b_kmajor, void* C, long long ldc,
                             int M, int N, int K, const float* bias1, const float* bias2,
                             int accumulate, int split_k, void* stream) {
    return gemm_go({dtype_in, dtype_out, A, lda, a_kmajor, B, ldb, b_kmajor, C, ldc, M, N, K, bias1, bias2, accumulate,
                    split_k, 0, nullptr, 0, false, nullptr}, false, stream);
}

extern "C" int edgedict_gemm_nt_lse(const void* A, long long lda, const void* B, long long ldb, void* C,
                                    long long ldc, int M, int N, int K, const float* bias,
                                    float* lse_part, void* stream) {
    ED_CHECK_ARG(A && B && C && lse_part, "gemm_nt_lse: null pointer");
    return gemm_go({ED_BF16, ED_BF16, A, lda, 1, B, ldb, 1, C, ldc, M, N, K, bias, nullptr, 0, 1, 0, nullptr, 0, false,
                    lse_part}, false, stream);
}

extern "C" int edgedict_gemm_bg(int dtype_in, int dtype_out, const void* A, long long lda,
                                int a_kmajor, const void* B, long long ldb, int b_kmajor, void* C,
                                long long ldc, int M, int N, int K, const float* bias1,
                                const float* bias2, int accumulate, int split_k,
                                int max_wg_per_cu, float* partials, void* stream) {
    return gemm_go({dtype_in, dtype_out, A, lda, a_kmajor, B, ldb, b_kmajor, C, ldc, M, N, K, bias1, bias2, accumulate,
                    split_k, max_wg_per_cu, partials, pow2_slices(split_k), false, nullptr}, true, stream);
}

extern "C" int edgedict_gemm_plan(int dtype_in, int dtype_out, const void* A, long long lda, int a_kmajor,
                                  const void* B, long long ldb, int b_kmajor, void* C, long long ldc, int M,
                                  int N, int K, const float* bias1, const float* bias2, int accumulate,
                                  int split_k, int max_wg_per_cu, float* partials, int lse, int unreduced,
                                  int32_t* record) {
    static float lse_dummy[2];
    ED_CHECK_ARG(record, "gemm_plan: null record");
    const GemmCall c = {dtype_in, dtype_out, A, lda, a_kmajor, B, ldb, b_kmajor, C, ldc, M, N, K, bias1, bias2, accumulate,
                        split_k, max_wg_per_cu, partials, unreduced ? 8 : pow2_slices(split_k), unreduced != 0,
                        lse ? lse_dummy : nullptr};
    GemmPlan p;
    int rc = gemm_validate(c, max_wg_per_cu != 0 && !unreduced);
    if (rc == ED_OK) rc = ed_gemm_plan(c, p);
    if (rc != ED_OK) return rc;
    const int32_t r[ED_GEMM_PLAN_WORDS] = {p.kernel, (int32_t)p.grid, p.block, p.lds, p.split, p.k_per_split,
                                           p.zero_first, p.reduce_after, p.vendor};
    for (int i = 0; i < ED_GEMM_PLAN_WORDS; ++i) record[i] = r[i];
    return ED_OK;
}
```

edgedict_amd/csrc/gemm_plan.hpp:

```cpp
#pragma once
#include <hip/hip_runtime.h>

struct GemmCall {
    int dtype_in, dtype_out;
    const void* A; long long lda; int a_kmajor;
    const void* B; long long ldb; int b_kmajor;
    void* C; long long ldc;
    int M, N, K;
    const float* bias1; const float* bias2;
    int accumulate, split_k;
    int max_wg_per_cu;
    float* partials;
    int slice_cap;
    bool unreduced;
    float* lse_part;
};

enum GemmKernel {
    ED_K_NONE = 0,
    ED_K_GENERIC_BF16_BF16 = 1, ED_K_GENERIC_BF16_BF16_FAST = 2,
    ED_K_GENERIC_BF16_F32 = 3, ED_K_GENERIC_BF16_F32_FAST = 4,
    ED_K_GENERIC_F32_F32 = 5, ED_K_GENERIC_F32_F32_FAST = 6,
    ED_K_NT_64 = 7, ED_K_NT_128 = 8, ED_K_NT_256X128 = 9,
    ED_K_NT_RING64 = 10,
    ED_K_NT256 = 11,
    ED_K_NT256R = 12, ED_K_NT256R_LSE = 13,
    ED_K_TN256 = 14,
};
enum GemmVendor { ED_VENDOR_NONE = 0, ED_VENDOR_NT_LOGITS = 1, ED_VENDOR_NT_SMALL = 2, ED_VENDOR_TN_F32 = 3 };

struct GemmPlan {
    int kernel;
    unsigned grid;
    int block, lds;
    int split, k_per_split;
    bool zero_first;
    bool reduce_after;
    int vendor;
};

constexpr int ED_NT256_LDS_BYTES = 128 * 1024, ED_NT256R_LDS_BYTES = 129 * 1024, ED_TN256_LDS_BYTES = 96 * 1024;

int ed_gemm_plan(const GemmCall& c, GemmPlan& p);
int ed_gemm_run(const GemmCall& c, const GemmPlan& p, hipStream_t s, int* slices = nullptr);

int ed_gemm_nt_launch(const GemmCall& c, const GemmPlan& p, hipStream_t s);
int ed_gemm_nt256_launch(const GemmCall& c, const GemmPlan& p, hipStream_t s);
int ed_gemm_nt256r_launch(const GemmCall& c, const GemmPlan& p, hipStream_t s);
int ed_gemm_tn256_launch(const GemmCall& c, const GemmPlan& p, hipStream_t s);
```

edgedict_amd/csrc/stack_kernels.hip:

```cpp
#include "stack_kernels.hpp"

#ifndef ED_STEP_PRIO
#define ED_STEP_PRIO 3
#endif
#ifndef ED_STACK_DBG
#define ED_STACK_DBG 0
#endif

namespace {

typedef __attribute__((ext_vector_type(8))) __bf16 bf16x8_t;
typedef __attribute__((ext_vector_type(4))) float f32x4_t;

__device__ __forceinline__ bf16x8_t ldfrag(const bf16_t* p) {
    uint4 v = *reinterpret_cast<const uint4*>(p);
    return *reinterpret_cast<bf16x8_t*>(&v);
}
__device__ __forceinline__ bf16x8_t zfrag() {
    uint4 v = make_uint4(0, 0, 0, 0);
    return *reinterpret_cast<bf16x8_t*>(&v);
}
__device__ __forceinline__ float fsigmoid(float x) { return __fdividef(1.f, 1.f + __expf(-x)); }
__device__ __forceinline__ float ftanh(float x) {
    const float xc = fminf(fmaxf(x, -15.f), 15.f);
// ... 1138 lines not shown
        asm volatile("s_waitcnt vmcnt(0)" ::: "memory");
        __syncthreads();
        if (tid == 0) __hip_atomic_fetch_add(cnt_arrive, 1u, __ATOMIC_RELAXED, __HIP_MEMORY_SCOPE_AGENT);
        SK_STAMP(4);
        if (live && !(ED_SK_TAIL & 1)) {
            bf16_t* G_t = S.G - (long long)s * B * H4 + (long long)crow * H4 + kc0;
#pragma unroll
            for (int i = 0; i < 2; ++i) *reinterpret_cast<u32x4_t*>(G_t + i * 16) = v16[i];
        }
        if (s + 1 < S.nsteps && !(ED_SK_TAIL & 2)) request_operands(s + 1);
        SK_STAMP(5);
    }
#undef SK_STAMP
    if (TRACE && tr) {
        long long* o = L.trace + S.layer * 8;
        for (int i = 0; i < 6; ++i) atomicAdd((unsigned long long*)(o + i), (unsigned long long)ph[i]);
        atomicAdd((unsigned long long*)(o + 6), (unsigned long long)S.nsteps);
        atomicAdd((unsigned long long*)(o + 7), 1ull);
    }
    if (live) *reinterpret_cast<float4*>(S.dC + (long long)crow * H + unit0) = dc;
    if (L.stamp) {
        __syncthreads();
        if (threadIdx.x == 0) atomicMax(&L.stamp[1], wall_clock64());
    }
}

__global__ void pack_whh_sk_kernel(const float* __restrict__ W, bf16_t* __restrict__ out, int H) {
    const long long n8 = 4ll * H * H / 8;
    const int KSq = H >> 5;
    for (long long c = (long long)blockIdx.x * blockDim.x + threadIdx.x; c < n8; c += (long long)gridDim.x * blockDim.x) {
        const int lane = (int)(c & 63), nn = (int)((c >> 6) & 3);
        const long long blk = c >> 8;
        const int ksl = (int)(blk % KSq), kq = (int)((blk / KSq) & 3), ub = (int)(blk / KSq / 4);
        const int unit = ub * 64 + nn * 16 + (lane & 15);
        const int kcol = kq * H + ksl * 32 + (lane >> 4) * 8;
        const int ubk = kcol >> 6, g = (kcol >> 4) & 3, u = kcol & 15;
        const float* src = W + ((long long)g * H + ubk * 16 + u) * H + unit;
        unsigned o[4];
#pragma unroll
        for (int e = 0; e < 4; ++e)
            o[e] = (unsigned)f32_to_bf16(src[(long long)(2 * e) * H]) | ((unsigned)f32_to_bf16(src[(long long)(2 * e + 1) * H]) << 16);
        *reinterpret_cast<uint4*>(out + c * 8) = make_uint4(o[0], o[1], o[2], o[3]);
    }
}

constexpr int LNB_NB = 4;
__global__ __launch_bounds__(256) void stack_ln_bwd_kernel(
    const bf16_t* __restrict__ dout, long long dout_st, long long dout_sb,
    const bf16_t* __restrict__ y, const bf16_t* __restrict__ res, const float* __restrict__ gamma,
    const float* __restrict__ mean_in, const float* __restrict__ rstd_in, bf16_t* __restrict__ dz,
    float* __restrict__ part, int B, int H, int t0, int t1, int reduce, unsigned drop_thresh, unsigned drop_seed,
    float drop_scale, int drop_T) {
    __shared__ float red[2][3][LNB_NB * 8][64];
    const int lane = threadIdx.x & 63, wave = threadIdx.x >> 6;
    const float scale = 1.f / (float)reduce;
    float ag[LNB_NB][8], ab[LNB_NB][8], gm[LNB_NB][8];
#pragma unroll
    for (int i = 0; i < LNB_NB; ++i) {
        const int c = lane * 8 + 512 * i;
#pragma unroll
        for (int e = 0; e < 8; ++e) {
            ag[i][e] = 0.f;
            ab[i][e] = 0.f;
            gm[i][e] = (c < H) ? gamma[c + e] : 0.f;
        }
    }
    const long long rows = (long long)(t1 - t0) * B;
    for (long long rr = (long long)blockIdx.x * 4 + wave; rr < rows; rr += (long long)gridDim.x * 4) {
        const int t = t0 + (int)(rr / B), b = (int)(rr % B);
        const long long row = (long long)t * B + b;
        const bf16_t* dyr = dout + (long long)(t / reduce) * dout_st + (long long)b * dout_sb;
        const bf16_t* yr = y + row * H;
        const bf16_t* rsr = res ? res + row * H : nullptr;
        const float m = mean_in[row], rs = rstd_in[row];
        float dy[LNB_NB][8], xh[LNB_NB][8];
        float s1 = 0.f, s2 = 0.f;
#pragma unroll
        for (int i = 0; i < LNB_NB; ++i) {
            const int c = lane * 8 + 512 * i;
            if (c < H) {
                float z[8];
                ElemIO<bf16_t>::load_vec(dyr + c, dy[i]);
                ElemIO<bf16_t>::load_vec(yr + c, z);
                if (rsr) {
                    float r2[8];
                    ElemIO<bf16_t>::load_vec(rsr + c, r2);
#pragma unroll
                    for (int e = 0; e < 8; ++e) z[e] += r2[e];
                }
                if (drop_thresh) {
                    const long long i0 = ((long long)b * drop_T + t / reduce) * H + c;
#pragma unroll
                    for (int e = 0; e < 8; ++e) dy[i][e] = ed_drop_keep(drop_seed, i0 + e, drop_thresh) ? dy[i][e] * drop_scale : 0.f;
                }
#pragma unroll
                for (int e = 0; e < 8; ++e) {
                    dy[i][e] *= scale;
                    xh[i][e] = (z[e] - m) * rs;
                    const float g = dy[i][e] * gm[i][e];
                    s1 += g;
                    s2 += g * xh[i][e];
                    ag[i][e] += dy[i][e] * xh[i][e];
                    ab[i][e] += dy[i][e];
                }
            }
        }
        s1 = wave_sum(s1) / (float)H;
        s2 = wave_sum(s2) / (float)H;
        bf16_t* dr = dz + row * H;
#pragma unroll
        for (int i = 0; i < LNB_NB; ++i) {
            const int c = lane * 8 + 512 * i;
            if (c < H) {
                float o[8];
#pragma unroll
                for (int e = 0; e < 8; ++e) o[e] = rs * (dy[i][e] * gm[i][e] - s1 - xh[i][e] * s2);
                ElemIO<bf16_t>::store_vec(dr + c, o);
            }
        }
    }
    if (wave > 0) {
#pragma unroll
        for (int i = 0; i < LNB_NB; ++i)
#pragma unroll
            for (int e = 0; e < 8; ++e) {
                red[0][wave - 1][i * 8 + e][lane] = ag[i][e];
                red[1][wave - 1][i * 8 + e][lane] = ab[i][e];
            }
    }
    __syncthreads();
    if (wave == 0) {
        float* pg = part + (long long)blockIdx.x * 2 * H;
        float* pb = pg + H;
#pragma unroll
        for (int i = 0; i < LNB_NB; ++i) {
            const int c = lane * 8 + 512 * i;
            if (c < H) {
                float og[8], ob[8];
#pragma unroll
                for (int e = 0; e < 8; ++e) {
                    const int k = i * 8 + e;
                    og[e] = ag[i][e] + red[0][0][k][lane] + red[0][1][k][lane] + red[0][2][k][lane];
                    ob[e] = ab[i][e] + red[1][0][k][lane] + red[1][1][k][lane] + red[1][2][k][lane];
                }
                *reinterpret_cast<float4*>(pg + c) = make_float4(og[0], og[1], og[2], og[3]);
                *reinterpret_cast<float4*>(pg + c + 4) = make_float4(og[4], og[5], og[6], og[7]);
                *reinterpret_cast<float4*>(pb + c) = make_float4(ob[0], ob[1], ob[2], ob[3]);
                *reinterpret_cast<float4*>(pb + c + 4) = make_float4(ob[4], ob[5], ob[6], ob[7]);
            }
        }
    }
}

__global__ __launch_bounds__(256) void stack_sum_parts_kernel(const float* __restrict__ part, int rows,
                                                             int H, float* __restrict__ dgamma,
                                                             float* __restrict__ dbeta) {
    const int c = blockIdx.x * 256 + threadIdx.x;
    if (c >= 2 * H) return;
    float a0 = 0.f, a1 = 0.f, a2 = 0.f, a3 = 0.f;
    int r = blockIdx.y;
    const int stride = gridDim.y;
    for (; r + 3 * stride < rows; r += 4 * stride) {
        a0 += part[(long long)r * 2 * H + c];
        a1 += part[(long long)(r + stride) * 2 * H + c];
        a2 += part[(long long)(r + 2 * stride) * 2 * H + c];
        a3 += part[(long long)(r + 3 * stride) * 2 * H + c];
    }
    for (; r < rows; r += stride) a0 += part[(long long)r * 2 * H + c];
    atomicAdd(c < H ? dgamma + c : dbeta + (c - H), (a0 + a1) + (a2 + a3));
}

template <typename T>
__global__ __launch_bounds__(256) void stack_input_norm_kernel(
    const T* __restrict__ x, const float* __restrict__ gamma, const float* __restrict__ beta,
    bf16_t* __restrict__ out, float* __restrict__ mean_out, float* __restrict__ rstd_out, int B,
    int Tn, int D, float eps) {
    const int lane = threadIdx.x & 63, wave = threadIdx.x >> 6;
    const long long rows = (long long)B * Tn;
    for (long long row = (long long)blockIdx.x * 4 + wave; row < rows; row += (long long)gridDim.x * 4) {
        const int b = (int)(row / Tn), t = (int)(row % Tn);
        const T* xr = x + row * D;
        float s = 0.f;
        for (int c = lane; c < D; c += 64) s += ElemIO<T>::load(xr + c);
        const float m = wave_sum(s) / (float)D;
        float v = 0.f;
        for (int c = lane; c < D; c += 64) {
            const float d = ElemIO<T>::load(xr + c) - m;
            v += d * d;
        }
        const float rs = rsqrtf(wave_sum(v) / (float)D + eps);
        if (lane == 0) {
            mean_out[row] = m;
            rstd_out[row] = rs;
        }
        bf16_t* o = out + ((long long)t * B + b) * D;
        for (int c = lane; c < D; c += 64)
            o[c] = f32_to_bf16((ElemIO<T>::load(xr + c) - m) * rs * gamma[c] + beta[c]);
    }
}

template <typename T>
__global__ __launch_bounds__(256) void stack_input_norm_bwd_kernel(
    const T* __restrict__ x, const bf16_t* __restrict__ dX, const float* __restrict__ mean_in,
    const float* __restrict__ rstd_in, float* __restrict__ dgamma, float* __restrict__ dbeta, int B,
    int Tn, int D, int rows_per_block) {
    const int c = threadIdx.x;
    if (c >= D) return;
    const long long rows = (long long)B * Tn;
    const long long r0 = (long long)blockIdx.x * rows_per_block;
    const long long r1 = min(rows, r0 + rows_per_block);
    float ag = 0.f, ab = 0.f;
    for (long long row = r0; row < r1; ++row) {
        const int t = (int)(row / B), b = (int)(row % B);
        const long long xrow = (long long)b * Tn + t;
        const float dy = bf16_to_f32(dX[row * D + c]);
        const float xh = (ElemIO<T>::load(x + xrow * D + c) - mean_in[xrow]) * rstd_in[xrow];
        ag += dy * xh;
        ab += dy;
    }
    atomicAdd(dgamma + c, ag);
    atomicAdd(dbeta + c, ab);
}

__global__ void stack_init_state_kernel(const float* __restrict__ h0, const float* __restrict__ c0,
                                        bf16_t* __restrict__ Yx0, float* __restrict__ Cx0,
                                        bf16_t* __restrict__ hfrag, int B, int H) {
    const int B16 = (B + 15) / 16 * 16;
    const long long n = (long long)B16 * H;
    for (long long i = (long long)blockIdx.x * blockDim.x + threadIdx.x; i < n;
         i += (long long)gridDim.x * blockDim.x) {
        const int b = (int)(i / H), j = (int)(i % H);
        const bool live = b < B;
        const bf16_t hv = f32_to_bf16((live && h0) ? h0[i] : 0.f);
        if (live) {
            Yx0[i] = hv;
            Cx0[i] = c0 ? c0[i] : 0.f;
        }
        hfrag[((((long long)(j >> 5) * (B16 >> 4) + (b >> 4)) * 64) + ((j & 31) >> 3) * 16 + (b & 15)) * 8 + (j & 7)] = hv;
    }
}

__global__ void stack_init_states_kernel(EdInitStates A) {
    const int l = blockIdx.y;
    const float* __restrict__ h0 = A.h0[l];
    const float* __restrict__ c0 = A.c0[l];
    bf16_t* __restrict__ Yx0 = A.Yx0[l];
    float* __restrict__ Cx0 = A.Cx0[l];
    bf16_t* __restrict__ hfrag = A.hfrag[l];
    const int B = A.B, H = A.H;
    const int B16 = (B + 15) / 16 * 16;
    const long long n = (long long)B16 * H;
    for (long long i = (long long)blockIdx.x * blockDim.x + threadIdx.x; i < n;
         i += (long long)gridDim.x * blockDim.x) {
        const int b = (int)(i / H), j = (int)(i % H);
        const bool live = b < B;
        const bf16_t hv = f32_to_bf16((live && h0) ? h0[i] : 0.f);
        if (live) {
            Yx0[i] = hv;
            Cx0[i] = c0 ? c0[i] : 0.f;
        }
        hfrag[((((long long)(j >> 5) * (B16 >> 4) + (b >> 4)) * 64) + ((j & 31) >> 3) * 16 + (b & 15)) * 8 + (j & 7)] = hv;
    }
}

}

int ed_stack_launch_fwd(const EdFwdLaunch& L, hipStream_t s) {
    const int UB = L.H >> 4, RG = (L.B + 63) >> 6, RB = (L.B + 3) >> 2;
    const int grid = L.nstep * UB * RG + L.nnorm * RB;
    if (grid == 0) return ED_OK;
    hipLaunchKernelGGL(stack_fwd_kernel, dim3(grid), dim3(256), 0, s, L);
    ED_CHECK_LAUNCH("stack_fwd_kernel");
    return ED_OK;
}

int ed_stack_multi_norm(const EdChunkNorm* items, int n, int B, int H, float eps, hipStream_t s) {
    if (n <= 0) return ED_OK;
    ED_CHECK_ARG(n <= ED_STACK_MAX_SLOTS, "stack_multi_norm: too many items");
    MultiNormArgs M;
    int grid = 0;
    M.n = 0;
    for (int i = 0; i < n; ++i) {
        const EdChunkNorm& e = items[i];
        if (e.t1 <= e.t0) continue;
        ChunkNormArgs& a = M.a[M.n];
        a.Yx1 = e.Yx1; a.X = e.X; a.gamma = e.gamma; a.beta = e.beta; a.out = e.out; a.out_st = e.out_st;
        a.out_sb = e.out_sb; a.mean = e.mean; a.rstd = e.rstd; a.B = B; a.H = H; a.T = e.T; a.t0 = e.t0;
        a.reduce = e.reduce; a.eps = eps;
        a.drop_thresh = e.drop_thresh; a.drop_seed = e.drop_seed; a.drop_scale = e.drop_scale; a.drop_T = e.drop_T;
        M.first[M.n] = grid;
        const int frames_out = e.reduce == 1 ? e.t1 - e.t0 : (e.t1 - e.t0 + 1) / 2;
        grid += frames_out * ((B + 3) >> 2);
        ++M.n;
    }
    M.first[M.n] = grid;
    if (grid == 0) return ED_OK;
    hipLaunchKernelGGL(stack_multi_norm_kernel, dim3(grid), dim3(256), 0, s, M);
    ED_CHECK_LAUNCH("stack_multi_norm_kernel");
    return ED_OK;
}

int ed_stack_wait_counters(const unsigned* const* counters, const unsigned* targets, int n, unsigned* err, hipStream_t s) {
    if (n <= 0) return ED_OK;
    ED_CHECK_ARG(n <= WAIT_COUNTERS_MAX, "stack_wait_counters: too many counters");
    WaitCountersArgs a;
    for (int i = 0; i < n; ++i) {
        a.counter[i] = counters[i];
        a.target[i] = targets[i];
    }
    a.n = n;
    a.err = err;
    hipLaunchKernelGGL(stack_wait_counters_kernel, dim3(1), dim3(64), 0, s, a);
    ED_CHECK_LAUNCH("stack_wait_counters_kernel");
    return ED_OK;
}

int ed_stack_sk_supported(int B, int H) { return (B >= 1 && B <= 64 && H % 64 == 0 && H >= 64 && H <= 1024) ? 1 : 0; }

int ed_stack_pack_sk(const float* w_hh, bf16_t* out, int H, hipStream_t s) {
    hipLaunchKernelGGL(pack_whh_sk_kernel, dim3(ed_grid_for(4ll * H * H / 8, 256, 4096)), dim3(256), 0, s, w_hh, out, H);
    ED_CHECK_LAUNCH("pack_whh_sk_kernel");
    return ED_OK;
}

int ed_stack_launch_bwd_sk(const EdSkLaunch& L, hipStream_t s) {
    const int grid = L.nslot * (L.H >> 6) * 4;
    if (grid == 0) return ED_OK;
    if (L.trace) hipLaunchKernelGGL(stack_bwd_sk_kernel<true>, dim3(grid), dim3(256), SK_RING * SK_SLOT, s, L);
    else hipLaunchKernelGGL(stack_bwd_sk_kernel<false>, dim3(grid), dim3(256), SK_RING * SK_SLOT, s, L);
    ED_CHECK_LAUNCH("stack_bwd_sk_kernel");
    return ED_OK;
}

int ed_stack_lpw_supported(int B, int H) {
    const int UB = H >> 4, RG = (B + 63) >> 6;
    return (H % 32 == 0 && (H >> 5) <= 4 * LPW_PER && UB * RG <= 64) ? 1 : 0;
}

int ed_stack_launch_fwd_lpw(const EdLpwLaunch& L, hipStream_t s) {
    const int UB = L.H >> 4, RG = (L.B + 63) >> 6;
    const int grid = L.nslot * UB * RG;
    if (grid == 0) return ED_OK;
#define ED_LPW_LAUNCH(TR, DPOLL) hipLaunchKernelGGL((stack_fwd_lpw_kernel<TR, DPOLL>), dim3(grid), dim3(256), 0, s, L)
    if (L.trace) { if (L.data_poll) ED_LPW_LAUNCH(true, true); else ED_LPW_LAUNCH(true, false); }
    else { if (L.data_poll) ED_LPW_LAUNCH(false, true); else ED_LPW_LAUNCH(false, false); }
#undef ED_LPW_LAUNCH
    ED_CHECK_LAUNCH("stack_fwd_lpw_kernel");
    return ED_OK;
}

int ed_stack_set_flag(unsigned* flag, hipStream_t s) {
    hipLaunchKernelGGL(stack_set_flag_kernel, dim3(1), dim3(64), 0, s, flag);
    ED_CHECK_LAUNCH("stack_set_flag_kernel");
    return ED_OK;
}

int ed_stack_launch_bwd(const EdBwdLaunch& L, hipStream_t s) {
    const int NB = L.H >> 5, RG = (L.B + 31) >> 5;
    const int grid = L.nstep * NB * RG;
    if (grid == 0) return ED_OK;
    hipLaunchKernelGGL(stack_bwd_kernel, dim3(grid), dim3(256), 0, s, L);
    ED_CHECK_LAUNCH("stack_bwd_kernel");
    return ED_OK;
}

int ed_stack_ln_bwd(const bf16_t* dout, long long dout_st, long long dout_sb, const bf16_t* y,
                    const bf16_t* res, const float* gamma, const float* mean, const float* rstd,
                    bf16_t* dz, float* part, int grid, int B, int H, int t0, int t1, int reduce,
                    hipStream_t s, unsigned drop_thresh, unsigned drop_seed, float drop_scale, int drop_T) {
    hipLaunchKernelGGL(stack_ln_bwd_kernel, dim3(grid), dim3(256), 0, s, dout, dout_st, dout_sb, y,
                       res, gamma, mean, rstd, dz, part, B, H, t0, max(t0, t1), reduce, drop_thresh, drop_seed,
                       drop_scale, drop_T);
    ED_CHECK_LAUNCH("stack_ln_bwd_kernel");
    return ED_OK;
}

int ed_stack_sum_parts(const float* part, int rows, int H, float* dgamma, float* dbeta, hipStream_t s) {
    if (rows <= 0) return ED_OK;
    const int gy = rows >= 64 ? 16 : 1;
    hipLaunchKernelGGL(stack_sum_parts_kernel, dim3((2 * H + 255) / 256, gy), dim3(256), 0, s, part,
                       rows, H, dgamma, dbeta);
    ED_CHECK_LAUNCH("stack_sum_parts_kernel");
    return ED_OK;
}

int ed_stack_input_norm(int x_dtype, const void* x, const float* gamma, const float* beta,
                        bf16_t* out, float* mean, float* rstd, int B, int T, int D, float eps,
                        hipStream_t s) {
    const int grid = ed_grid_for((long long)B * T, 4, 256 * 16);
    if (x_dtype == ED_F32)
        hipLaunchKernelGGL(stack_input_norm_kernel<float>, dim3(grid), dim3(256), 0, s,
                           (const float*)x, gamma, beta, out, mean, rstd, B, T, D, eps);
    else
        hipLaunchKernelGGL(stack_input_norm_kernel<bf16_t>, dim3(grid), dim3(256), 0, s,
                           (const bf16_t*)x, gamma, beta, out, mean, rstd, B, T, D, eps);
    ED_CHECK_LAUNCH("stack_input_norm_kernel");
    return ED_OK;
}

int ed_stack_input_norm_bwd(int x_dtype, const void* x, const bf16_t* dX, const float* mean,
                            const float* rstd, float* dgamma, float* dbeta, int B, int T, int D,
                            hipStream_t s) {
    const long long rows = (long long)B * T;
    const int rpb = 64;
    const int grid = (int)((rows + rpb - 1) / rpb);
    const int threads = (D + 63) / 64 * 64;
    if (x_dtype == ED_F32)
        hipLaunchKernelGGL(stack_input_norm_bwd_kernel<float>, dim3(grid), dim3(threads), 0, s,
                           (const float*)x, dX, mean, rstd, dgamma, dbeta, B, T, D, rpb);
    else
        hipLaunchKernelGGL(stack_input_norm_bwd_kernel<bf16_t>, dim3(grid), dim3(threads), 0, s,
                           (const bf16_t*)x, dX, mean, rstd, dgamma, dbeta, B, T, D, rpb);
    ED_CHECK_LAUNCH("stack_input_norm_bwd_kernel");
    return ED_OK;
}

int ed_stack_init_state(const float* h0, const float* c0, bf16_t* Yx0, float* Cx0, bf16_t* hfrag,
                        int B, int H, hipStream_t s) {
    const long long n = (long long)((B + 15) / 16 * 16) * H;
    hipLaunchKernelGGL(stack_init_state_kernel, dim3(ed_grid_for(n, 256)), dim3(256), 0, s, h0, c0,
                       Yx0, Cx0, hfrag, B, H);
    ED_CHECK_LAUNCH("stack_init_state_kernel");
    return ED_OK;
}

int ed_stack_init_states(const EdInitStates& A, hipStream_t s) {
    if (A.n <= 0) return ED_OK;
    ED_CHECK_ARG(A.n <= 8, "stack_init_states: too many layers in one call");
    const long long n = (long long)((A.B + 15) / 16 * 16) * A.H;
    hipLaunchKernelGGL(stack_init_states_kernel, dim3(ed_grid_for(n, 256), A.n), dim3(256), 0, s, A);
    ED_CHECK_LAUNCH("stack_init_states_kernel");
    return ED_OK;
}

int ed_stack_zero(void* p, size_t bytes, hipStream_t s) {
    ED_CHECK_HIP(hipMemsetAsync(p, 0, bytes, s));
    return ED_OK;
}
```

edgedict_amd/csrc/stack_kernels.hpp:

```cpp
#pragma once
#include "common.hpp"

constexpr int ED_STACK_MAX_SLOTS = 8;

__host__ __device__ inline int ed_gate_col(int gate, int j) {
    return (j >> 4) * 64 + gate * 16 + (j & 15);
}

struct EdFwdStep {
    bf16_t* G_t;
    const bf16_t* hfrag_in;
    bf16_t* hfrag_out;
    bf16_t* Y_t;
    const float* C_prev;
    float* C_t;
    const bf16_t* Wfrag;
    const unsigned* wait_flag;
};

struct EdFwdNorm {
    const bf16_t* y0;
    const bf16_t* r0;
    const bf16_t* y1;
    const bf16_t* r1;
    const float* gamma;
    const float* beta;
    bf16_t* out;
    long long out_stride;
    float* mean0; float* rstd0;
    float* mean1; float* rstd1;
    float scale;
    unsigned drop_thresh, drop_seed;
    float drop_scale;
    int drop_T, tau;
};

struct EdFwdLaunch {
    EdFwdStep step[ED_STACK_MAX_SLOTS];
    EdFwdNorm norm[ED_STACK_MAX_SLOTS];
    int nstep, nnorm;
    int B, H;
    float eps;
    unsigned long long* stamp;
    unsigned* err;
};

struct EdBwdStep {
    bf16_t* G_t;
    const bf16_t* gfrag_in;
    bf16_t* gfrag_out;
    const bf16_t* dY_t;
    const float* C_t;
    const float* C_prev;
    float* dC;
    const bf16_t* WTfrag;
    const unsigned* wait_flag;
};

struct EdBwdLaunch {
    EdBwdStep step[ED_STACK_MAX_SLOTS];
    int nstep;
    int B, H;
    unsigned long long* stamp;
    unsigned* err;
};

struct EdLpwSlot {
    bf16_t* G;
    bf16_t* img;
    long long img_stride;
    long long img_bytes;
    bf16_t* Y;
    const float* C_prev;
    float* C;
    const bf16_t* Wfrag;
    unsigned* counter;
    unsigned base;
    const unsigned* wait_flag;
    int t0, nsteps;
    int layer;
};
constexpr int LPW_CNT_STRIDE = 64;
struct EdLpwLaunch {
    EdLpwSlot slot[ED_STACK_MAX_SLOTS];
    int nslot;
    int data_poll;
    int B, H;
    unsigned long long* stamp;
    unsigned* err;
    long long* trace;
};
int ed_stack_launch_fwd_lpw(const EdLpwLaunch& L, hipStream_t s);
struct EdChunkNorm {
    const bf16_t* Yx1;
    const bf16_t* X;
    const float* gamma;
    const float* beta;
    bf16_t* out;
    long long out_st, out_sb;
    float* mean;
    float* rstd;
    int T, t0, t1, reduce;
    unsigned drop_thresh, drop_seed;
    float drop_scale;
    int drop_T;
};
int ed_stack_wait_counters(const unsigned* const* counters, const unsigned* targets, int n, unsigned* err, hipStream_t s);
int ed_stack_multi_norm(const EdChunkNorm* items, int n, int B, int H, float eps, hipStream_t s);
int ed_stack_lpw_supported(int B, int H);

constexpr int SK_CNT_QUARTER = 16;
constexpr int SK_CNT_LINES = 32;
struct EdSkSlot {
    bf16_t* G;
    bf16_t* img;
    long long img_stride, img_bytes;
    const bf16_t* dY;
    const float* Cx;
    float* dC;
    const bf16_t* Wsk;
    float* part;
    unsigned* counter;
    unsigned* gcounter;
    unsigned done;
    const unsigned* wait_flag;
    int t0, nsteps, T, layer;
};
struct EdSkLaunch {
    EdSkSlot slot[ED_STACK_MAX_SLOTS];
    int nslot;
    int B, H;
    unsigned long long* stamp;
    unsigned* err;
    long long* trace;
};
int ed_stack_launch_bwd_sk(const EdSkLaunch& L, hipStream_t s);
int ed_stack_sk_supported(int B, int H);
int ed_stack_pack_sk(const float* w_hh, bf16_t* out, int H, hipStream_t s);

int ed_stack_launch_fwd(const EdFwdLaunch& L, hipStream_t s);
int ed_stack_set_flag(unsigned* flag, hipStream_t s);
int ed_stack_launch_bwd(const EdBwdLaunch& L, hipStream_t s);
int ed_stack_ln_bwd(const bf16_t* dout, long long dout_st, long long dout_sb, const bf16_t* y,
                    const bf16_t* res, const float* gamma, const float* mean, const float* rstd,
                    bf16_t* dz, float* part, int grid, int B, int H, int t0, int t1, int reduce,
                    hipStream_t s, unsigned drop_thresh = 0, unsigned drop_seed = 0, float drop_scale = 1.f,
                    int drop_T = 0);
int ed_stack_sum_parts(const float* part, int rows, int H, float* dgamma, float* dbeta, hipStream_t s);
int ed_stack_input_norm(int x_dtype, const void* x, const float* gamma, const float* beta,
                        bf16_t* out, float* mean, float* rstd, int B, int T, int D, float eps,
                        hipStream_t s);
int ed_stack_input_norm_bwd(int x_dtype, const void* x, const bf16_t* dX, const float* mean,
                            const float* rstd, float* dgamma, float* dbeta, int B, int T, int D,
                            hipStream_t s);
struct EdInitStates {
    int n, B, H;
    const float* h0[8];
    const float* c0[8];
    bf16_t* Yx0[8];
    float* Cx0[8];
    bf16_t* hfrag[8];
};
int ed_stack_init_states(const EdInitStates& A, hipStream_t s);
int ed_stack_init_state(const float* h0, const float* c0, bf16_t* Yx0, float* Cx0, bf16_t* hfrag,
                        int B, int H, hipStream_t s);
int ed_stack_zero(void* p, size_t bytes, hipStream_t s);
```

edgedict_amd/encoder_stack.py:

```python
import ctypes
import os
import weakref

import torch

from . import _lib, config, ops, side
from ._lib import check, dtype_code, ptr, stream_ptr

F32 = torch.float32
BF16 = torch.bfloat16
_vp, _fp = ctypes.c_void_p, ctypes.c_void_p


class StackLayer(ctypes.Structure):
    _fields_ = [("T", ctypes.c_int), ("I", ctypes.c_int), ("reduce", ctypes.c_int),
                ("residual", ctypes.c_int),
                ("wih_p", _vp), ("wih_t", _vp), ("bias_p", _fp), ("whh_f", _vp), ("whh_b", _vp),
                ("ln_gamma", _fp), ("ln_beta", _fp),
                ("X", _vp), ("G", _vp), ("Yx", _vp), ("Cx", _fp), ("mean", _fp), ("rstd", _fp),
                ("dZ", _vp), ("dX", _vp), ("dW_ih", _fp), ("dW_hh", _fp), ("db", _fp), ("db_hh", _fp),
                ("dgamma", _fp), ("dbeta", _fp), ("whh_s", _vp),
                ("drop_p", ctypes.c_float), ("drop_seed", ctypes.c_uint)]


class StackDesc(ctypes.Structure):
    _fields_ = [("B", ctypes.c_int), ("H", ctypes.c_int), ("L", ctypes.c_int),
                ("chunk", ctypes.c_int), ("lag", ctypes.c_int), ("split_k", ctypes.c_int),
                ("flags", ctypes.c_int), ("eps", ctypes.c_float),
                ("layers", ctypes.POINTER(StackLayer)),
                ("x", _vp), ("x_dtype", ctypes.c_int), ("T0", ctypes.c_int), ("I0", ctypes.c_int),
                ("in_gamma", _fp), ("in_beta", _fp), ("in_mean", _fp), ("in_rstd", _fp),
                ("h0", _fp), ("c0", _fp), ("out", _vp), ("dout", _vp),
                ("d_in_gamma", _fp), ("d_in_beta", _fp), ("ws", _vp), ("ws_bytes", ctypes.c_size_t),
                ("grads_final", _vp), ("grads_final_user", _vp)]


GRADS_FINAL_CB = ctypes.CFUNCTYPE(None, ctypes.c_int, ctypes.c_void_p)


SERIAL = 1
DW_AT_END = 2
ACCUM_GRADS = 8
INFERENCE = 64

CHUNK = int(os.environ.get("EDGEDICT_STACK_CHUNK", "16"))
LAG = int(os.environ.get("EDGEDICT_STACK_LAG", "0"))
SPLIT_K = int(os.environ.get("EDGEDICT_STACK_SPLITK", "0"))
FLAGS = int(os.environ.get("EDGEDICT_STACK_FLAGS", "0"))
BWD_SK = os.environ.get("EDGEDICT_STACK_BWD_SK_PACK", "1") != "0"


def _p(t):
    return None if t is None else t.data_ptr()


def supported(cd, H, I0, L, reductions):
    return (cd == BF16 and H % 32 == 0 and 32 <= H <= 2048 and I0 % 8 == 0 and 8 <= I0 <= 1024
            and 1 <= L <= 8 and all(r in (1, 2) for r in reductions) and config.USE_ENCODER_STACK)


class _PackedLayer:
    __slots__ = ("key", "bwd_key", "ref", "wih_p", "wih_t", "bias_p", "whh_f", "whh_b", "whh_s")

    def __init__(self, owner):
        self.key = self.bwd_key = None
        self.ref = weakref.ref(owner)


_PACKED = {}


def _sources(*ts):
    srcs = [t.detach().contiguous() for t in ts]
    for t in srcs:
        if t.dtype != F32:
            raise TypeError("encoder stack: master weights must be fp32")
    return srcs


def packed_weights(w_ih, w_hh, b_ih, b_hh, backward_images=True):
    ent = _PACKED.get(id(w_hh))
    key = (w_ih.data_ptr(), w_hh.data_ptr(), w_ih._version, w_hh._version, b_ih._version,
           b_hh._version, config.param_epoch(), BWD_SK)
    if ent is None or ent.ref() is not w_hh or ent.key != key:
        for k in [k for k, v in _PACKED.items() if v.ref() is None]:
            del _PACKED[k]
        ent = _PACKED[id(w_hh)] = _PackedLayer(w_hh)
        H4, I = w_ih.shape
        H = H4 // 4
        dev = w_ih.device
        srcs = _sources(w_ih, w_hh, b_ih, b_hh)
        ent.wih_p = torch.empty(H4, I, dtype=BF16, device=dev)
        ent.wih_t = torch.empty(I, H4, dtype=BF16, device=dev)
        ent.bias_p = torch.empty(H4, dtype=F32, device=dev)
        ent.whh_f = torch.empty(H4 * H, dtype=BF16, device=dev)
        ent.whh_b = torch.empty(H4 * H, dtype=BF16, device=dev)
        ent.whh_s = torch.empty(H4 * H, dtype=BF16, device=dev) if (BWD_SK and H % 64 == 0 and 64 <= H <= 1024) else None
        check(_lib.load().edgedict_stack_pack_weights(ptr(srcs[0]), ptr(srcs[1]), ptr(srcs[2]), ptr(srcs[3]),
                                                      H, I, ptr(ent.wih_p), None, ptr(ent.bias_p), ptr(ent.whh_f),
                                                      None, stream_ptr()), "stack_pack_weights")
        ent.key = key
    if backward_images:
        fill_backward_images(ent, w_ih, w_hh)
    return ent


def fill_backward_images(ent, w_ih, w_hh):
    if ent.bwd_key == ent.key:
        return
    H4, I = w_ih.shape
    H = H4 // 4
    srcs = _sources(w_ih, w_hh)
    lib = _lib.load()
    check(lib.edgedict_stack_pack_weights(ptr(srcs[0]), ptr(srcs[1]), None, None, H, I, None, ptr(ent.wih_t), None,
                                          None, ptr(ent.whh_b), stream_ptr()), "stack_pack_weights (backward images)")
    if ent.whh_s is not None:
        check(lib.edgedict_stack_pack_sk(ptr(srcs[1]), H, ptr(ent.whh_s), stream_ptr()), "stack_pack_sk")
    ent.bwd_key = ent.key


def clear_cache():
    _PACKED.clear()


def check_wsr_error():
    code = _lib.load().edgedict_stack_wsr_error()
    if 500 <= code < 700:
        raise RuntimeError("edgedict_amd: a step kernel of the encoder stack gave up waiting for a chunk product "
                           "of the side stream (code %d: %s pass, launch slot %d); the results of that call are "
                           "garbage. EDGEDICT_STACK_SOFT_WAIT=0 orders the streams with events instead"
                           % (code, "forward" if code < 600 else "backward", code % 100))
    if code:
        raise RuntimeError("edgedict_amd: a launch-persistent encoder launch gave up waiting for its peers (code %d); "
                           "the results of that call are garbage. EDGEDICT_STACK_LPW=0 / EDGEDICT_STACK_BWD_SK=0 "
                           "select the launch-per-step kernels (e.g. when two processes share the device)" % code)


def last_mode(backward):
    kind, steps = ctypes.c_int(-1), ctypes.c_int(-1)
    check(_lib.load().edgedict_stack_last_mode(1 if backward else 0, ctypes.byref(kind), ctypes.byref(steps)),
          "stack_last_mode")
    return kind.value, steps.value


_PREPACK_EVENT = [None, None]


def prepack(encoder, stream):
    lstm = encoder.lstm
    if not hasattr(lstm, "lstms"):
        return
    with torch.cuda.stream(stream):
        ents = [(packed_weights(*m.layer(0), backward_images=False), m.layer(0)) for m in lstm.lstms]
        _PREPACK_EVENT[0] = stream.record_event()
        for ent, lay in ents:
            fill_backward_images(ent, lay[0], lay[1])
        _PREPACK_EVENT[1] = stream.record_event()


class _Plan:

    def __init__(self, x, in_norm, layers, reductions, h0, c0, flags, drop=None):
        self.keep = []
        if _PREPACK_EVENT[0] is not None:
            torch.cuda.current_stream(x.device).wait_event(_PREPACK_EVENT[0])
            _PREPACK_EVENT[0] = None
        B, T0, I0 = x.shape
        dev = x.device
        L = len(layers)
        H = layers[0][1].shape[1]
        self.B, self.H, self.L, self.T0, self.I0 = B, H, L, T0, I0
        self.x = x
        self.in_mean = torch.empty(B * T0, dtype=F32, device=dev)
        self.in_rstd = torch.empty(B * T0, dtype=F32, device=dev)
        self.larr = (StackLayer * L)()
        self.layer_bufs = []
        self.packs = []
        T, I = T0, I0
        for l, (w_ih, w_hh, b_ih, b_hh, ln_w, ln_b) in enumerate(layers):
            pk = packed_weights(w_ih, w_hh, b_ih, b_hh, backward_images=False)
            self.packs.append((pk, w_ih, w_hh))
            bufs = dict(
                X=torch.empty(T, B, I, dtype=BF16, device=dev),
                G=torch.empty(T, B, 4 * H, dtype=BF16, device=dev),
                Yx=torch.empty(T + 1, B, H, dtype=BF16, device=dev),
                Cx=torch.empty(T + 1, B, H, dtype=F32, device=dev),
                mean=torch.empty(T, B, dtype=F32, device=dev),
                rstd=torch.empty(T, B, dtype=F32, device=dev))
            self.layer_bufs.append(bufs)
            y = self.larr[l]
            y.T, y.I, y.reduce, y.residual = T, I, reductions[l], int(l != 0)
            y.wih_p, y.wih_t, y.bias_p, y.whh_f, y.whh_b = map(
                _p, (pk.wih_p, pk.wih_t, pk.bias_p, pk.whh_f, pk.whh_b))
            y.whh_s = _p(pk.whh_s)
            y.drop_p, y.drop_seed = (float(drop[0]), int(drop[1][l]) & 0xFFFFFFFF) if drop else (0.0, 0)
            g, b = ln_w.detach(), ln_b.detach()
            y.ln_gamma, y.ln_beta = _p(g), _p(b)
            self.keep += [pk.wih_p, pk.wih_t, pk.bias_p, pk.whh_f, pk.whh_b, pk.whh_s, g, b]
            for k, v in bufs.items():
                setattr(y, k, _p(v))
            T = (T + reductions[l] - 1) // reductions[l]
            I = H
        self.T_out = T
        self.out = torch.empty(B, T, H, dtype=BF16, device=dev)
        d = self.desc = StackDesc()
        d.B, d.H, d.L = B, H, L
        d.chunk, d.lag, d.split_k, d.flags, d.eps = CHUNK, LAG, SPLIT_K, flags, 1e-5
        d.layers = ctypes.cast(self.larr, ctypes.POINTER(StackLayer))
        d.x, d.x_dtype, d.T0, d.I0 = _p(x), dtype_code(x.dtype), T0, I0
        ig, ib = in_norm[0].detach(), in_norm[1].detach()
        self.keep += [ig, ib, h0, c0]
        d.in_gamma, d.in_beta = _p(ig), _p(ib)
        d.in_mean, d.in_rstd = _p(self.in_mean), _p(self.in_rstd)
        d.h0, d.c0 = _p(h0), _p(c0)
        d.out = _p(self.out)
        lib = _lib.load()
        d.ws, d.ws_bytes = None, 0
        n = lib.edgedict_stack_workspace_bytes(ctypes.byref(d))
        self.ws = torch.empty(n, dtype=torch.uint8, device=dev)
        d.ws, d.ws_bytes = _p(self.ws), n

    def forward(self):
        lib = _lib.load()
        check_wsr_error()
        ops.mark("stack_fwd:enter")
        with ops.host_timed("stack_forward_call"):
            check(lib.edgedict_stack_forward(ctypes.byref(self.desc), stream_ptr()), "stack_forward")
        ops.mark("stack_fwd:exit")

    def final_states(self):
        hN = torch.stack([b["Yx"][-1] for b in self.layer_bufs], 0).float()
        cN = torch.stack([b["Cx"][-1] for b in self.layer_bufs], 0).clone()
        return hN, cN

    def backward(self, dout, params, in_norm, all_trainable=True):
        dev = dout.device
        B, H = self.B, self.H
        grads = []
        d = self.desc
        if _PREPACK_EVENT[1] is not None:
            torch.cuda.current_stream(dev).wait_event(_PREPACK_EVENT[1])
            _PREPACK_EVENT[1] = None
        for pk, w_ih, w_hh in self.packs:
            fill_backward_images(pk, w_ih, w_hh)
        everyone = list(params) + list(in_norm)
        direct = all_trainable and config.DEFER_WEIGHT_GRADS and all(side.accumulates_in_place(p) for p in everyone)
        zeros = None if direct else torch.zeros(2 * H * self.L + 2 * self.I0, dtype=F32, device=dev)
        for l in range(self.L):
            y = self.larr[l]
            T, I = y.T, y.I
            w_ih, w_hh, b_ih, b_hh, ln_w, ln_b = params[6 * l:6 * l + 6]
            dZ = torch.empty(T, B, H, dtype=BF16, device=dev)
            gb = dict(dZ=dZ, dX=dZ if y.residual else (torch.empty(T, B, I, dtype=BF16, device=dev)
                                                       if l > 0 else None))
            if direct:
                gb.update(dW_ih=w_ih.grad, dW_hh=w_hh.grad, db=b_ih.grad, db_hh=b_hh.grad,
                          dgamma=ln_w.grad, dbeta=ln_b.grad)
            else:
                gb.update(dW_ih=torch.empty(4 * H, I, dtype=F32, device=dev),
                          dW_hh=torch.empty(4 * H, H, dtype=F32, device=dev),
                          db=torch.empty(4 * H, dtype=F32, device=dev), db_hh=None,
                          dgamma=zeros[2 * H * l:2 * H * l + H],
                          dbeta=zeros[2 * H * l + H:2 * H * (l + 1)])
            for k, v in gb.items():
                setattr(y, k, _p(v))
            grads.append(gb)
        if direct:
            dig, dib = in_norm[0].grad, in_norm[1].grad
            d.flags |= ACCUM_GRADS
        else:
            dig = zeros[2 * H * self.L:2 * H * self.L + self.I0]
            dib = zeros[2 * H * self.L + self.I0:]
            d.flags &= ~ACCUM_GRADS
        dout = dout.contiguous()
        d.dout, d.d_in_gamma, d.d_in_beta = _p(dout), _p(dig), _p(dib)
        from . import dp
        cb = None
        if direct and dp.READY_HOOK is not None:
            hook, aux = dp.READY_HOOK, side.stream(dev)

            errors = []

            def _on_final(layer, _user, params=params, hook=hook, aux=aux):
                try:
                    hook(params[6 * layer:6 * layer + 4], aux)
                except BaseException as exc:
                    errors.append(exc)
            cb = GRADS_FINAL_CB(_on_final)
            d.grads_final = ctypes.cast(cb, ctypes.c_void_p).value
        else:
            d.grads_final = None
        d.grads_final_user = None
        lib = _lib.load()
        ops.mark("stack_bwd:enter")
        with ops.host_timed("stack_backward_call"):
            check(lib.edgedict_stack_backward(ctypes.byref(d), stream_ptr()), "stack_backward")
        d.grads_final = None
        if cb is not None and errors:
            raise errors[0]
        ops.mark("stack_bwd:exit")
        return None if direct else (dig, dib, grads)


class EncoderStackFn(torch.autograd.Function):

    @staticmethod
    def forward(ctx, xs, in_g, in_b, h0, c0, reductions, flags, drop, *params):
        assert len(params) % 6 == 0
        layers = [params[i:i + 6] for i in range(0, len(params), 6)]
        x = xs.contiguous()
        if x.dtype not in (F32, BF16):
            x = x.float()
        needs_bwd = any(ctx.needs_input_grad)
        plan = _Plan(x, (in_g, in_b), layers, list(reductions), h0, c0,
                     (FLAGS if flags is None else flags) | (0 if needs_bwd else INFERENCE), drop)
        with ops.timed("enc_stack_fwd_T%d_L%d" % (x.shape[1], len(layers))):
            plan.forward()
        hN, cN = plan.final_states()
        out, plan.out = plan.out, None
        ctx.plan = plan
        ctx.params = params
        ctx.in_norm = (in_g, in_b)
        ctx.mark_non_differentiable(hN, cN)
        return out, hN, cN

    @staticmethod
    def backward(ctx, dout, _dh, _dc):
        plan = ctx.plan
        if plan is None:
            raise RuntimeError("edgedict_amd: the encoder stack's saved activations were consumed "
                               "by a previous backward (retain_graph is not supported)")
        ctx.plan = None
        if dout.dtype != BF16:
            dout = dout.to(BF16)
        with ops.timed("enc_stack_bwd_T%d_L%d" % (plan.T0, plan.L)):
            trainable = all(ctx.needs_input_grad[1:3]) and all(ctx.needs_input_grad[8:])
            res = plan.backward(dout, ctx.params, ctx.in_norm, trainable)
        if res is None:
            return (None,) * (8 + len(ctx.params))
        dig, dib, grads = res
        out = [None, dig, dib, None, None, None, None, None]
        for gb in grads:
            out += [gb["dW_ih"], gb["dW_hh"], gb["db"], gb["db"].clone(), gb["dgamma"], gb["dbeta"]]
        return tuple(out)


def schedule(T0, I0, H, reductions, B=64, chunk=None, backward=False, lag=0, flags=0, grads_final=None):
    import numpy as np
    lib = _lib.load()
    L = len(reductions)
    chunk = chunk or CHUNK
    layers = (StackLayer * L)()
    dummy = ctypes.c_void_p(0x1000)
    fdummy = ctypes.cast(dummy, _fp)
    T, I = T0, I0
    Ts = []
    for l in range(L):
        y = layers[l]
        y.T, y.I, y.reduce, y.residual = T, I, reductions[l], 1 if l > 0 else 0
        for name, typ in StackLayer._fields_[4:]:
            if typ in (_vp, _fp):
                setattr(y, name, fdummy if typ is _fp else dummy)
        y.drop_p, y.drop_seed = 0.0, 0
        Ts.append(T)
        T = (T + reductions[l] - 1) // reductions[l]
        I = H
    d = StackDesc()
    d.B, d.H, d.L, d.chunk, d.lag, d.split_k, d.flags, d.eps = B, H, L, chunk, lag, 0, flags, 1e-5
    d.layers = layers
    d.x, d.x_dtype, d.T0, d.I0 = dummy, 1, T0, I0
    for name in ("in_gamma", "in_beta", "in_mean", "in_rstd", "d_in_gamma", "d_in_beta"):
        setattr(d, name, fdummy)
    d.h0 = d.c0 = None
    d.out = d.dout = d.ws = dummy
    d.ws_bytes = 1 << 62
    cb = None
    if grads_final is not None:
        cb = GRADS_FINAL_CB(lambda layer, _user: grads_final(layer))
        d.grads_final = ctypes.cast(cb, ctypes.c_void_p).value
    f0 = 1
    for r in reductions:
        f0 *= r
    fl, f = [], f0
    for l in range(L):
        fl.append(f)
        f //= reductions[l]
    nch = [(Ts[l] + chunk * fl[l] - 1) // (chunk * fl[l]) for l in range(L)]
    steps = np.full(sum(Ts), -2, dtype=np.int32)
    enq = np.full(sum(nch), -2, dtype=np.int32)
    nl, ms = ctypes.c_int32(0), ctypes.c_int32(0)
    rc = lib.edgedict_stack_schedule(ctypes.byref(d), 1 if backward else 0,
                                     steps.ctypes.data_as(ctypes.c_void_p), enq.ctypes.data_as(ctypes.c_void_p),
                                     ctypes.byref(nl), ctypes.byref(ms))
    _lib.check(rc, "stack_schedule")
    so = np.cumsum([0] + Ts)
    co = np.cumsum([0] + nch)
    return ([steps[so[l]:so[l + 1]] for l in range(L)], [enq[co[l]:co[l + 1]] for l in range(L)],
            int(nl.value), int(ms.value))
```

include/edgedict_hip.h:

```cpp
#ifndef EDGEDICT_HIP_H
#define EDGEDICT_HIP_H

#include <stddef.h>
#include <stdint.h>

#ifdef __cplusplus
extern "C" {
#endif

#define EDGEDICT_ABI_VERSION 1

#define ED_OK 0
#define ED_ERR_INVALID (-1)
#define ED_ERR_LAUNCH (-2)

#define ED_F32 0
#define ED_BF16 1

const char* edgedict_last_error(void);
int edgedict_abi_version(void);

size_t edgedict_rnnt_workspace_bytes(int B, int T, int U1);
int edgedict_rnnt_loss_forward(const void* acts, int acts_dtype, const int32_t* labels,
                               const int32_t* act_lens, const int32_t* label_lens, int B, int T,
// ... 70 lines not shown
                                  const int32_t* label_lens, const int32_t* win_lo, const int32_t* win_hi, int B, int T,
                                  int U1, int V, int blank, float* costs, float* reduced, float reduce_scale,
                                  void* workspace, void* stream);
int edgedict_rnnt_loss_forward_packed_ar(const void* acts, int acts_dtype, const int32_t* labels,
                                         const int32_t* act_lens, const int32_t* label_lens, const int32_t* win_lo,
                                         const int32_t* win_hi, const long long* row_offsets, int B, int T, int U1, int V,
                                         int blank, float* costs, float* reduced, float reduce_scale, void* workspace,
                                         void* stream);
int edgedict_rnnt_loss_forward_packed_parts_ar(const void* acts, const int32_t* labels, const int32_t* act_lens,
                                               const int32_t* label_lens, const int32_t* win_lo, const int32_t* win_hi,
                                               const long long* row_offsets, int B, int T, int U1, int V, int blank,
                                               float* costs, float* reduced, float reduce_scale, void* workspace,
                                               const float* lse_parts, int lse_slots, void* stream);
int edgedict_rnnt_loss_backward_ar(const void* acts, int acts_dtype, void* grads, const int32_t* labels,
                                   const int32_t* act_lens, const int32_t* label_lens, int B, int T, int U1, int V,
                                   int blank, const void* workspace, float grad_scale_host,
                                   const float* grad_scale_dev, int grad_scale_stride, float fastemit_lambda,
                                   void* stream);
int edgedict_rnnt_loss_backward_packed_ar(const void* acts, int acts_dtype, void* grads, const int32_t* labels,
                                          const int32_t* act_lens, const int32_t* label_lens,
                                          const long long* row_offsets, int B, int T, int U1, int V, int blank,
                                          const void* workspace, float grad_scale_host, const float* grad_scale_dev,
                                          int grad_scale_stride, float fastemit_lambda, void* stream);
int edgedict_rnnt_loss_backward_packed_colsum_ar(const void* acts, int acts_dtype, void* grads, const int32_t* labels,
                                                 const int32_t* act_lens, const int32_t* label_lens,
                                                 const long long* row_offsets, int B, int T, int U1, int V, int blank,
                                                 const void* workspace, float grad_scale_host,
                                                 const float* grad_scale_dev, int grad_scale_stride,
                                                 float* colsum_parts, float fastemit_lambda, void* stream);
int edgedict_rnnt_loss_backward_packed_range_ar(const void* acts, int acts_dtype, void* grads, const int32_t* labels,
                                                const int32_t* act_lens, const int32_t* label_lens,
                                                const long long* row_offsets, int B, int T, int U1, int V, int blank,
                                                const void* workspace, float grad_scale_host,
                                                const float* grad_scale_dev, int grad_scale_stride, int b0, int nb,
                                                float fastemit_lambda, void* stream);
int edgedict_rnnt_align_ar(const void* acts, int acts_dtype, const int32_t* labels, const int32_t* act_lens,
                           const int32_t* label_lens, const int32_t* win_lo, const int32_t* win_hi, int B, int T, int U1,
                           int V, int blank, int32_t* frames, float* scores, void* workspace, void* stream);
int edgedict_rnnt_align_packed_ar(const void* acts, int acts_dtype, const int32_t* labels, const int32_t* act_lens,
                                  const int32_t* label_lens, const int32_t* win_lo, const int32_t* win_hi,
                                  const long long* row_offsets, int B, int T, int U1, int V, int blank, int32_t* frames,
                                  float* scores, void* workspace, void* stream);
int edgedict_rnnt_align_packed_parts_ar(const void* acts, const int32_t* labels, const int32_t* act_lens,
                                        const int32_t* label_lens, const int32_t* win_lo, const int32_t* win_hi,
                                        const long long* row_offsets, int B, int T, int U1, int V, int blank,
                                        int32_t* frames, float* scores, void* workspace, const float* lse_parts,
                                        int lse_slots, void* stream);
int edgedict_rnnt_alignment_windows(const int32_t* frames, const int32_t* act_lens, const int32_t* label_lens, int B,
                                    int T, int U, int left, int right, int32_t* win_lo, int32_t* win_hi, void* stream);
int edgedict_rnnt_band(const int32_t* win_lo, const int32_t* win_hi, const int32_t* act_lens, const int32_t* label_lens,
                       int B, int T, int U1, int32_t* band, long long* cells, void* stream);
int edgedict_rnnt_band_offsets(const int32_t* band, const long long* cells, int B, int T, long long* row_off,
                               long long* total, void* stream);
int edgedict_rnnt_band_rows(const int32_t* band, const long long* row_off, int B, int T, int U1, long long rows,
                            int32_t* row_tu, void* stream);
int edgedict_rnnt_loss_forward_band(const void* acts, int acts_dtype, const int32_t* labels, const int32_t* act_lens,
                                    const int32_t* label_lens, const int32_t* win_lo, const int32_t* win_hi,
                                    const int32_t* band, const long long* row_off, const int32_t* row_tu,
                                    const long long* cells, int B, int T, int U1, int V, int blank, float* costs,
                                    float* reduced, float reduce_scale, void* workspace, void* stream);
int edgedict_rnnt_loss_forward_band_parts(const void* acts, const int32_t* labels, const int32_t* act_lens,
                                          const int32_t* label_lens, const int32_t* win_lo, const int32_t* win_hi,
                                          const int32_t* band, const long long* row_off, const int32_t* row_tu,
                                          const long long* cells, int B, int T, int U1, int V, int blank, float* costs,
                                          float* reduced, float reduce_scale, void* workspace, const float* lse_parts,
                                          int lse_slots, void* stream);
int edgedict_rnnt_loss_backward_band(const void* acts, int acts_dtype, void* grads, const int32_t* labels,
                                     const int32_t* act_lens, const int32_t* label_lens, const long long* row_off,
                                     const int32_t* row_tu, const long long* cells, int B, int T, int U1, int V, int blank,
                                     const void* workspace, float grad_scale_host, const float* grad_scale_dev,
                                     int grad_scale_stride, float fastemit_lambda, void* stream);
int edgedict_rnnt_loss_backward_band_colsum(const void* acts, int acts_dtype, void* grads, const int32_t* labels,
                                            const int32_t* act_lens, const int32_t* label_lens, const long long* row_off,
                                            const int32_t* row_tu, const long long* cells, int B, int T, int U1, int V,
                                            int blank, const void* workspace, float grad_scale_host,
                                            const float* grad_scale_dev, int grad_scale_stride, float* colsum_parts,
                                            float fastemit_lambda, void* stream);
const void* edgedict_rnnt_workspace_view(const void* workspace, int B, int T, int U1, int which);

int edgedict_gemm(int dtype_in, int dtype_out, const void* A, long long lda, int a_kmajor,
                  const void* B, long long ldb, int b_kmajor, void* C, long long ldc, int M, int N,
                  int K, const float* bias1, const float* bias2, int accumulate, int split_k,
                  void* stream);

int edgedict_gemm_bg(int dtype_in, int dtype_out, const void* A, long long lda, int a_kmajor,
                     const void* B, long long ldb, int b_kmajor, void* C, long long ldc, int M,
                     int N, int K, const float* bias1, const float* bias2, int accumulate,
                     int split_k, int max_wg_per_cu, float* partials, void* stream);

int edgedict_gemm_nt_lse(const void* A, long long lda, const void* B, long long ldb, void* C,
                         long long ldc, int M, int N, int K, const float* bias, float* lse_part,
                         void* stream);

#define ED_GEMM_PLAN_WORDS 9
int edgedict_gemm_plan(int dtype_in, int dtype_out, const void* A, long long lda, int a_kmajor,
                       const void* B, long long ldb, int b_kmajor, void* C, long long ldc, int M, int N,
                       int K, const float* bias1, const float* bias2, int accumulate, int split_k,
                       int max_wg_per_cu, float* partials, int lse, int unreduced, int32_t* record);


int edgedict_layernorm_fwd(int dtype, const void* x, const void* res, const float* gamma,
                           const float* beta, void* y, float* mean, float* rstd, int B, int T,
                           int D, int reduce, float eps, void* stream);
int edgedict_layernorm_bwd(int dtype, const void* dout, const void* x, const void* res,
                           const float* gamma, const float* mean, const float* rstd, void* ds,
                           float* dgamma, float* dbeta, int B, int T, int D, int reduce,
                           void* stream);

size_t edgedict_lstm_workspace_bytes(int dtype, int B, int H);
int edgedict_lstm_pack_weights(int src_dtype, const void* Whh, void* packed_fwd, void* packed_bwd,
                               int H, void* stream);
int edgedict_lstm_forward(int dtype, void* G, void* Hprev, void* Y, float* Cst, const void* Whh,
                          const void* Whh_packed, const float* h0, const float* c0, float* hN,
                          float* cN, int B, int T, int H, void* ws, void* stream);
int edgedict_lstm_backward(int dtype, void* G, const void* dY, const float* Cst, const float* c0,
                           const void* WhhT, const void* WhhT_packed, float* dC_ws, int B, int T,
                           int H, void* ws, void* stream);

typedef struct edgedict_stack_layer {
    int T;
    int I;
    int reduce;
    int residual;
    const void* wih_p;
    const void* wih_t;
    const float* bias_p;
    const void* whh_f;
    const void* whh_b;
    const float* ln_gamma;
    const float* ln_beta;
    void* X;
    void* G;
    void* Yx;
    float* Cx;
    float* mean;
    float* rstd;
    void* dZ;
    void* dX;
    float* dW_ih;
    float* dW_hh;
    float* db;
    float* db_hh;
    float* dgamma;
    float* dbeta;
    const void* whh_s;
    float drop_p;
    unsigned drop_seed;
} edgedict_stack_layer_t;

#define EDGEDICT_STACK_SERIAL 1
#define EDGEDICT_STACK_DW_AT_END 2
#define EDGEDICT_STACK_ACCUM_GRADS 8
#define EDGEDICT_STACK_INFERENCE 64
#define EDGEDICT_STACK_SIDE_STREAM_PER_LAYER 4

typedef struct edgedict_stack_desc {
    int B, H, L;
    int chunk;
    int lag;
    int split_k;
    int flags;
    float eps;
    const edgedict_stack_layer_t* layers;
    const void* x;
    int x_dtype, T0, I0;
    const float* in_gamma;
    const float* in_beta;
    float* in_mean;
    float* in_rstd;
    const float* h0;
    const float* c0;
    void* out;
    const void* dout;
    float* d_in_gamma;
    float* d_in_beta;
    void* ws;
    size_t ws_bytes;
    void (*grads_final)(int layer, void* user);
    void* grads_final_user;
} edgedict_stack_desc_t;

size_t edgedict_stack_struct_bytes(int which);
void* edgedict_aux_stream(int which);
int edgedict_streams_busy(unsigned* mask);
size_t edgedict_stack_workspace_bytes(const edgedict_stack_desc_t* desc);
int edgedict_stack_pack_weights(const float* w_ih, const float* w_hh, const float* b_ih,
                                const float* b_hh, int H, int I, void* wih_p, void* wih_t,
                                float* bias_p, void* whh_f, void* whh_b, void* stream);
int edgedict_stack_pack_sk(const float* w_hh, int H, void* whh_s, void* stream);
int edgedict_stack_wsr_error(void);
void* edgedict_stack_error_words(int host);
int edgedict_stack_wsr_set_trace(void* device_buffer);
int edgedict_stack_forward(const edgedict_stack_desc_t* desc, void* stream);
int edgedict_stack_last_timing(int backward, float* ms, int* launches);
int edgedict_stack_last_mode(int backward, int* kind, int* steps_per_launch);
int edgedict_stack_time_launches(int on);
int edgedict_stack_launch_times(int backward, float* sum_ms, int* launches);
int edgedict_stack_launch_stamps(int backward, unsigned long long* out, int max_launches, int* launches);
int edgedict_stack_schedule(const edgedict_stack_desc_t* d, int backward, int32_t* step_launch,
                            int32_t* chunk_enqueued, int32_t* n_launches, int32_t* max_slots);
int edgedict_stack_backward(const edgedict_stack_desc_t* desc, void* stream);

int edgedict_cast(int src_dtype, const void* src, int dst_dtype, void* dst, long long n,
                  void* stream);
int edgedict_transpose(int src_dtype, const void* src, int dst_dtype, void* dst, int R, int C,
                       void* stream);
int edgedict_colsum(int dtype, const void* x, long long ld, float* out, long long M, int N,
                    void* stream);
int edgedict_embedding_fwd(int out_dtype, int emb_dtype, const int32_t* tokens, int tok_stride,
                           const void* emb, void* out, int B, int Uout, int E, int V,
                           int prepend_bos, int bos, void* stream);
int edgedict_embedding_bwd(int dtype, const int32_t* tokens, int tok_stride, const void* dout,
                           float* demb, int B, int Uout, int E, int V, int prepend_bos, int bos,
                           int pad, void* stream);
int edgedict_dropout(int dtype, const void* x, void* y, long long n, float p, unsigned seed,
                     void* stream);
int edgedict_spec_mask(float* x, int B, int T, int F, const int32_t* t_iv, int n_t,
                       const int32_t* f_iv, int n_f, void* stream);
int edgedict_joint_hidden_fwd(int dtype, const void* E1, const void* D1, void* hid, int B, int T,
                              int U1, int J, void* stream);
int edgedict_joint_hidden_bwd(int dtype, const void* dhid, const void* hid, float* dE1,
                              float* dD1, int B, int T, int U1, int J, void* stream);
int edgedict_joint_hidden_fwd_packed(int dtype, const void* E1, const void* D1, void* hid,
                                     const int32_t* act_lens, const int32_t* label_lens,
                                     const long long* row_offsets, int B, int T, int U1, int J,
                                     void* stream);
int edgedict_joint_hidden_bwd_packed(int dtype, const void* dhid, const void* hid, float* dE1,
                                     float* dD1, const int32_t* act_lens, const int32_t* label_lens,
                                     const long long* row_offsets, int B, int T, int U1, int J,
                                     void* stream);
int edgedict_joint_hidden_fwd_band(int dtype, const void* E1, const void* D1, void* hid, const int32_t* band,
                                   const long long* row_off, long long rows, int B, int T, int U1, int J, void* stream);
int edgedict_joint_hidden_bwd_band(int dtype, const void* dhid, const void* hid, float* dE1, float* dD1,
                                   const int32_t* band, const long long* row_off, long long rows, int B, int T, int U1,
                                   int J, void* stream);

int edgedict_adam_step(float* p, const float* g, float* m, float* v, long long n, float lr,
                       float beta1, float beta2, float eps, int step, float weight_decay,
                       float grad_scale_host, const float* grad_scale, void* p_bf16, void* stream);
int edgedict_adam_step_guarded(float* p, const float* g, float* m, float* v, long long n, float lr,
                               float beta1, float beta2, float eps, int step, float weight_decay,
                               float grad_scale_host, const float* grad_scale, void* p_bf16,
                               const unsigned* skip_words, int n_skip, unsigned* guard_scratch,
                               void* stream);
int edgedict_grad_clip_coef(const float* g, long long n, float max_norm, float pre_scale,
                            float* sumsq_ws, float* coef, float* norm_out, void* stream);
int edgedict_debug_footprint(float* buf, long long n_floats, int workgroups, int passes, void* stream);

int edgedict_dither(float* wave, long long wave_stride, int B, int N, const int32_t* lengths,
                    float amplitude, unsigned seed, void* stream);
int edgedict_fbank_forward(const float* wave, long long wave_stride, int B, int N,
                           const int32_t* lengths, const float* window, const float* twiddle,
                           const float* fb, const int32_t* fb_range, int n_fft, int win_lo,
                           int win_hi, int hop, int n_mels, float preemph, int do_log, void* out,
                           int out_dtype, long long o_b, long long o_group, long long o_k,
                           long long o_m, int stack, int frames_out, void* stream);
int edgedict_fbank_forward_masked(const float* wave, long long wave_stride, int B, int N,
                                  const int32_t* seq_len, const float* window,
                                  const float* twiddle, const float* fb, const int32_t* fb_range,
                                  int n_fft, int win_lo, int win_hi, int hop, int n_mels,
                                  float preemph, int do_log, float* out, long long o_b,
                                  long long o_m, int frames_out, int copies, long long o_copy,
                                  int normalize, int n_signal, void* stream);

size_t edgedict_greedy_workspace_bytes(int dtype, int B, int J, int V, int E, int L, int H, int P2);
int edgedict_greedy_decode(int dtype, const void* E1, long long e_row_stride,
                           long long e_frame_stride, int B, int T, int J, const void* W1d,
                           long long ldw1, const float* b1, int P2, const void* W2,
                           const float* b2, int V, const void* emb, int emb_dtype, int E, int L,
                           const void* const* w_ih, const void* const* w_hh,
                           const float* const* b_ih, const float* const* b_hh, int H,
                           const void* Wp, const float* bp, float* h_state, float* c_state,
                           void* dec_out, int blank, int unk, int32_t* tokens_out, int tok_stride,
                           float* score, void* workspace, void* stream);

int edgedict_gru_forward(int dtype, void* G, void* Hprev, void* Y, void* HN, const void* Whh,
                         const float* b_hh, const float* h0, float* hN, int B, int T, int H,
                         void* stream);
int edgedict_gru_backward(int dtype, void* G, void* DH, const void* dY, const void* Hprev,
                          const void* HN, const void* WhhT, float* dh_ws, int B, int T, int H,
                          void* stream);

int edgedict_conv_out_frames(int Tin, int k, int s);
int edgedict_conv_im2col(int in_dtype, int out_dtype, const void* x, void* cols, int B, int Tin, int C,
                         int k, int s, void* stream);
int edgedict_conv_col2im(int dtype, const void* dcols, void* dx, int B, int Tin, int C, int k, int s,
                         void* stream);
int edgedict_gelu_groupnorm_fwd(int dtype, const void* y, const float* gamma, const float* beta,
                                void* out, float* mean, float* rstd, int B, int T, int C, float eps,
                                void* stream);
size_t edgedict_gelu_groupnorm_bwd_workspace_bytes(int B, int T, int C);
int edgedict_gelu_groupnorm_bwd(int dtype, const void* y, const void* dout, const float* gamma,
                                const float* mean, const float* rstd, void* dy, float* dgamma,
                                float* dbeta, void* workspace, int B, int T, int C, void* stream);

long long edgedict_blaslt_calls(void);

size_t edgedict_stream_encoder_workspace_bytes(int B, int T, int I0, int H, int L);
int edgedict_stream_encoder_step(const void* xs, int x_dtype, int B, int T, int I0, int H, int L,
                                 const float* in_gamma, const float* in_beta, const void* const* w_ih,
                                 const void* const* w_hh, const float* const* b_ih, const float* const* b_hh,
                                 const float* const* ln_gamma, const float* const* ln_beta, const int* reduce,
                                 float* h_state, float* c_state, void* out, int* T_out, void* workspace,
                                 void* stream);

size_t edgedict_beam_workspace_bytes(int dtype, int B, int T, int J, int V, int E, int L, int H,
// ... 239 lines not shown
```

Baseline: 3377 utterances/s.

## Compute input-norm gamma/beta grads via G^T·xhat GEMM instead of full dX0

Drops the full dX0 = G·W_ih GEMM over all T·B rows that existed only to feed the input layer-norm backward. The forward pass now saves xhat with an appended ones column. In backward, G^T·[xhat,1] is formed as a 4H×(I0+8) product on a side stream and contracted with W_ih to give dgamma and dbeta. The per-layer LN partial sums are batched into one launch issued earlier, and the layer-0/1 bias colsum moves onto a side stream. This costs extra workspace for xhat and partials, and the gradients are reassociated in a different order.

```diff
diff --git a/edgedict_amd/csrc/encoder_stack.hip b/edgedict_amd/csrc/encoder_stack.hip
--- a/edgedict_amd/csrc/encoder_stack.hip
+++ b/edgedict_amd/csrc/encoder_stack.hip
@@ -9,7 +9,8 @@
 
 int ed_gemm_quiet_partials(int dtype_in, const void* A, long long lda, int a_kmajor, const void* B,
                            long long ldb, int b_kmajor, int M, int N, int K, int split_k,
-                           int max_wg_per_cu, float* partials, int* slices, hipStream_t stream);
+                           int max_wg_per_cu, float* partials, int* slices, hipStream_t stream,
+                           bool beside = false);
 
 namespace {
 
@@ -260,13 +261,17 @@
     std::vector<size_t> gimg;
     size_t gimg_stride = 0;
     std::vector<size_t> skpart;
-    size_t tmpW = 0, tmpB = 0, dX0 = 0, wsr_sync = 0, total = 0;
+    size_t tmpW = 0, tmpB = 0, tmpB0 = 0, xhat = 0, tmpS = 0, inpart = 0, wsr_sync = 0, total = 0;
 };
 constexpr size_t SYNC_FFLAG = 0, SYNC_BFLAG = 8 * 512, SYNC_FCNT = 2 * 8 * 512;
 constexpr size_t SYNC_BCNT = SYNC_FCNT + (size_t)8 * LPW_CNT_STRIDE;
 constexpr size_t SYNC_GCNT = 16 * 1024;
 constexpr size_t WSR_SYNC_BYTES = (SYNC_GCNT + (size_t)8 * SK_CNT_LINES * 64) * 4;
 static_assert(SYNC_BCNT + (size_t)8 * LPW_CNT_STRIDE <= SYNC_GCNT, "sync region layout");
+
+bool in_norm_grad_live(const edgedict_stack_desc_t* d) {
+    return !(d->flags & (EDGEDICT_STACK_INFERENCE | EDGEDICT_STACK_INPUT_NORM_FROZEN));
+}
 
 WsLayout ws_layout(const edgedict_stack_desc_t* d) {
     WsLayout w;
@@ -296,7 +301,13 @@
     }
     w.tmpW = off; off += align256((size_t)8 * 4 * d->H * maxK * sizeof(float));
     w.tmpB = off; off += align256((size_t)4 * d->H * sizeof(float));
-    w.dX0 = off; off += align256((size_t)d->T0 * d->B * d->I0 * sizeof(bf16_t));
+    w.tmpB0 = off; off += align256((size_t)2 * 4 * d->H * sizeof(float));
+    w.xhat = off;
+    if (in_norm_grad_live(d)) off += align256((size_t)d->T0 * d->B * (d->I0 + 8) * sizeof(bf16_t));
+    w.tmpS = off;
+    if (in_norm_grad_live(d)) off += align256((size_t)8 * 4 * d->H * (d->I0 + 8) * sizeof(float));
+    w.inpart = off;
+    if (in_norm_grad_live(d)) off += align256(ed_stack_input_norm_grad_part_bytes(d->H, d->I0));
     w.wsr_sync = off; off += WSR_SYNC_BYTES;
     w.himg_stride = align256(B16 * d->H * sizeof(bf16_t));
     for (int l = 0; l < d->L; ++l) {
@@ -823,7 +834,8 @@
     }
 
     ED_DEV(ed_stack_input_norm(d->x_dtype, d->x, d->in_gamma, d->in_beta, bptr(d->layers[0].X),
-                               d->in_mean, d->in_rstd, B, d->T0, d->I0, d->eps, st.C));
+                               in_norm_grad_live(d) ? bptr(ws + wl.xhat) : nullptr, d->in_mean, d->in_rstd, B, d->T0,
+                               d->I0, d->eps, st.C));
     const int lpw_ns = lpw_steps(d);
     if (lpw_ns && (poison_on() || lpw_data_poll()))
         ED_DEV(ed_stack_fill(ws + wl.himg[0], 0xff,
@@ -1151,7 +1163,7 @@
 extern "C" int edgedict_stack_backward(const edgedict_stack_desc_t* d, void* stream_) {
     std::vector<Geom> g;
     ED_TRY(validate(d, g, true));
-    ED_CHECK_ARG(d->dout && d->d_in_gamma && d->d_in_beta, "encoder_stack: null backward pointer in descriptor");
+    ED_CHECK_ARG(d->dout, "encoder_stack: null backward pointer in descriptor");
     ED_CHECK_ARG(!(d->flags & EDGEDICT_STACK_INFERENCE), "encoder_stack: backward on a descriptor flagged EDGEDICT_STACK_INFERENCE");
     const int B = d->B, H = d->H, L = d->L;
     const long long BH = (long long)B * H;
@@ -1211,9 +1223,29 @@
             else ED_TRY(st.record(Eb[L - 1][k], S));
         }
     }
+    auto sum_ln_parts = [&](hipStream_t S) -> int {
+        for (int l = 0; l < L; ++l) ED_TRY(st.chain(st.S[l], S));
+        EdSumParts A;
+        A.n = L;
+        A.H = H;
+        for (int l = 0; l < L; ++l) {
+            A.part[l] = (const float*)(ws + wl.lnpart[l]);
+            A.rows[l] = g[l].nchunks * LNB_GRID;
+            A.gy[l] = 0;
+            A.dgamma[l] = d->layers[l].dgamma;
+            A.dbeta[l] = d->layers[l].dbeta;
+        }
+        ED_DEV(ed_stack_sum_parts(A, S));
+        return ED_OK;
+    };
+    if (L == 1) ED_TRY(sum_ln_parts(st.S[0]));
     std::vector<int> deferred;
 
     const int acc_grads = (d->flags & EDGEDICT_STACK_ACCUM_GRADS) ? 1 : 0;
+    const bool in_grad = in_norm_grad_live(d) && (d->d_in_gamma || d->d_in_beta);
+    int side_env = 1, db_env = 2;
+    if (const char* e = getenv("EDGEDICT_STACK_INNORM_SIDE")) side_env = atoi(e);
+    if (const char* e = getenv("EDGEDICT_STACK_DB_SIDE")) db_env = atoi(e);
     auto weight_grads = [&](int l, int t0, int t1, bool first, bool last_of_all) -> int {
         if (g_trace) {
             if (t0 == 0 && d->grads_final) d->grads_final(l, d->grads_final_user);
@@ -1228,17 +1260,39 @@
         const int cap = last_of_all ? 4 : 2;
         const int acc = (acc_grads || !first) ? 1 : 0;
         int S = 1;
+        auto bias_grad = [&](hipStream_t sb, float* tb) -> int {
+            ED_TRY(ed_stack_zero(tb, (size_t)4 * H * sizeof(float), sb));
+            ED_TRY(edgedict_colsum(ED_BF16, bptr(y.G) + r0 * 4 * H, 4ll * H, tb, M, 4 * H, sb));
+            hipLaunchKernelGGL(unpermute_rows_kernel, dim3(ed_grid_for(4ll * H, 256, 4096)), dim3(256),
+                               0, sb, tb, 0, 1, y.db, y.db_hh, H, 1, acc);
+            ED_CHECK_LAUNCH("unpermute_rows_kernel");
+            return ED_OK;
+        };
+        const bool side = l == 0 && side_env != 0;
+        const bool db_side = (l == 0 && db_env != 0) || (l == 1 && first && t0 == 0 && db_env > 1);
+        hipEvent_t ev_db = nullptr;
+        if (db_side || (side && in_grad)) ED_TRY(st.chain(st.RS(l), st.S[l]));
+        if (db_side) {
+            ED_TRY(bias_grad(st.S[l], (float*)(ws + wl.tmpB0) + (size_t)l * 4 * H));
+            ED_TRY(st.record(ev_db, st.S[l]));
+        }
+        if (l == 0 && in_grad) {
+            const int N1 = d->I0 + 8;
+            float* tmpS = (float*)(ws + wl.tmpS);
+            hipStream_t s = side ? st.S[0] : st.W;
+            ED_TRY(ed_gemm_quiet_partials(ED_BF16, bptr(y.G) + r0 * 4 * H, 4ll * H, 0, bptr(ws + wl.xhat) + r0 * N1, N1,
+                                          0, 4 * H, N1, M, sk, cap, tmpS, &S, s, side));
+            ED_TRY(ed_stack_input_norm_grad(tmpS, 4ll * H * N1, S, bptr(y.wih_p), H, d->I0, (float*)(ws + wl.inpart),
+                                            d->d_in_gamma, d->d_in_beta, s));
+        }
         ED_TRY(ed_gemm_quiet_partials(ED_BF16, bptr(y.G) + r0 * 4 * H, 4ll * H, 0, bptr(y.X) + r0 * y.I, y.I, 0,
                                       4 * H, y.I, M, sk, cap, tmpW, &S, st.W));
         ED_TRY(unpermute_rows(tmpW, 4ll * H * y.I, S, y.dW_ih, nullptr, H, y.I, acc, st.W));
         ED_TRY(ed_gemm_quiet_partials(ED_BF16, bptr(y.G) + r0 * 4 * H, 4ll * H, 0, bptr(y.Yx) + r0 * H, H, 0,
                                       4 * H, H, M, sk, cap, tmpW, &S, st.W));
         ED_TRY(unpermute_rows(tmpW, 4ll * H * H, S, y.dW_hh, nullptr, H, H, acc, st.W));
-        ED_TRY(ed_stack_zero(tmpB, (size_t)4 * H * sizeof(float), st.W));
-        ED_TRY(edgedict_colsum(ED_BF16, bptr(y.G) + r0 * 4 * H, 4ll * H, tmpB, M, 4 * H, st.W));
-        hipLaunchKernelGGL(unpermute_rows_kernel, dim3(ed_grid_for(4ll * H, 256, 4096)), dim3(256),
-                           0, st.W, tmpB, 0, 1, y.db, y.db_hh, H, 1, acc);
-        ED_CHECK_LAUNCH("unpermute_rows_kernel");
+        if (db_side) ED_TRY(st.wait(st.W, ev_db));
+        else ED_TRY(bias_grad(st.W, tmpB));
         if (t0 == 0 && d->grads_final) d->grads_final(l, d->grads_final_user);
         return ED_OK;
     };
@@ -1276,6 +1330,7 @@
                 queued[l - 1][k] = 1;
                 ready_w[l - 1][k] = w + margin;
                 if (g_trace) g_trace->chunk_enqueued[g_trace->coff[l - 1] + k] = g_trace->launches;
+                if (l == 1 && k == 0) ED_TRY(sum_ln_parts(S));
             }
             const int k_split = (l <= 1 && tail_split > 1 && g[l].nchunks >= 2 * tail_split && dw_seg >= g[l].nchunks &&
                                  !(d->flags & EDGEDICT_STACK_DW_AT_END))
@@ -1446,22 +1501,6 @@
         ED_CHECK_HIP(hipEventRecord(st.rt->tev[1][1], st.R));
         st.rt->tlaunches[1] = Wtot;
     }
-    {
-        const edgedict_stack_layer_t& y = d->layers[0];
-        bf16_t* dX0 = bptr(ws + wl.dX0);
-        ED_TRY(st.chain(st.RS(0), st.S[0]));
-        ED_DEV(edgedict_gemm(ED_BF16, ED_BF16, y.G, 4ll * H, 1, y.wih_t ? y.wih_t : y.wih_p,
-                             y.wih_t ? 4ll * H : y.I, y.wih_t ? 1 : 0, dX0, y.I, y.T * B, y.I, 4 * H,
-                             nullptr, nullptr, 0, 1, st.S[0]));
-        ED_DEV(ed_stack_input_norm_bwd(d->x_dtype, d->x, dX0, d->in_mean, d->in_rstd, d->d_in_gamma,
-                                       d->d_in_beta, B, d->T0, d->I0, st.S[0]));
-        for (int l = 1; l < L; ++l) ED_TRY(st.chain(st.S[l], st.S[0]));
-        for (int l = 0; l < L; ++l) {
-            const edgedict_stack_layer_t& z = d->layers[l];
-            const float* part = (const float*)(ws + wl.lnpart[l]);
-            ED_DEV(ed_stack_sum_parts(part, g[l].nchunks * LNB_GRID, H, z.dgamma, z.dbeta, st.S[0]));
-        }
-    }
     if (!deferred.empty()) {
         ED_TRY(st.chain(st.R, st.W));
         if (st.R2 != st.R) ED_TRY(st.chain(st.R2, st.W));
diff --git a/edgedict_amd/csrc/gemm.hip b/edgedict_amd/csrc/gemm.hip
--- a/edgedict_amd/csrc/gemm.hip
+++ b/edgedict_amd/csrc/gemm.hip
@@ -432,7 +432,7 @@
     }
     const bool dw = c.dtype_in == ED_BF16 && c.dtype_out == ED_F32 && !c.a_kmajor && !c.b_kmajor &&
                     (long long)M * N >= (1ll << 18);
-    if (dw && c.partials && K >= 1024 && tn256_ok(c)) {
+    if (dw && c.partials && K >= 1024 && tn256_ok(c) && !c.beside) {
         const long long tiles = (long long)((M + 255) / 256) * ((N + 127) / 128);
         long long s = n_cu / tiles < c.slice_cap ? n_cu / tiles : c.slice_cap;
         while (s > 1 && s * 8 > (K + 31) / 32) --s;
@@ -452,7 +452,7 @@
         return ED_OK;
     }
     if (dw && (c.max_wg_per_cu > 0 || c.partials) && !has_bias && K >= 4096 && c.lda % 8 == 0 && c.ldb % 8 == 0 &&
-        c.ldc % 4 == 0)
+        c.ldc % 4 == 0 && !c.beside)
         p.vendor = ED_VENDOR_TN_F32;
     const bool f32 = c.dtype_in == ED_F32;
     const int bk = f32 ? 16 : 64, vec = f32 ? 4 : 8, ktiles = (K + bk - 1) / bk;
@@ -562,10 +562,10 @@
 
 int ed_gemm_quiet_partials(int dtype_in, const void* A, long long lda, int a_kmajor, const void* B,
                            long long ldb, int b_kmajor, int M, int N, int K, int split_k,
-                           int max_wg_per_cu, float* partials, int* slices, hipStream_t stream) {
+                           int max_wg_per_cu, float* partials, int* slices, hipStream_t stream, bool beside) {
     ED_CHECK_ARG(partials, "gemm: quiet product without a partials buffer");
     return gemm_go({dtype_in, ED_F32, A, lda, a_kmajor, B, ldb, b_kmajor, partials, N, M, N, K, nullptr, nullptr, 0, split_k,
-                    max_wg_per_cu, partials, 8, true, nullptr}, false, stream, slices);
+                    max_wg_per_cu, partials, 8, true, nullptr, beside}, false, stream, slices);
 }
 
 extern "C" int edgedict_gemm(int dtype_in, int dtype_out, const void* A, long long lda, int a_kmajor,
diff --git a/edgedict_amd/csrc/gemm_plan.hpp b/edgedict_amd/csrc/gemm_plan.hpp
--- a/edgedict_amd/csrc/gemm_plan.hpp
+++ b/edgedict_amd/csrc/gemm_plan.hpp
@@ -14,6 +14,7 @@
     int slice_cap;
     bool unreduced;
     float* lse_part;
+    bool beside;
 };
 
 enum GemmKernel {
diff --git a/edgedict_amd/csrc/stack_kernels.hip b/edgedict_amd/csrc/stack_kernels.hip
--- a/edgedict_amd/csrc/stack_kernels.hip
+++ b/edgedict_amd/csrc/stack_kernels.hip
@@ -1314,14 +1314,15 @@
     }
 }
 
-__global__ __launch_bounds__(256) void stack_sum_parts_kernel(const float* __restrict__ part, int rows,
-                                                             int H, float* __restrict__ dgamma,
-                                                             float* __restrict__ dbeta) {
+__global__ __launch_bounds__(256) void stack_sum_parts_kernel(EdSumParts A) {
+    const int l = blockIdx.z;
+    const int H = A.H, rows = A.rows[l];
+    const float* __restrict__ part = A.part[l];
     const int c = blockIdx.x * 256 + threadIdx.x;
-    if (c >= 2 * H) return;
+    if (c >= 2 * H || (int)blockIdx.y >= A.gy[l]) return;
     float a0 = 0.f, a1 = 0.f, a2 = 0.f, a3 = 0.f;
     int r = blockIdx.y;
-    const int stride = gridDim.y;
+    const int stride = A.gy[l];
     for (; r + 3 * stride < rows; r += 4 * stride) {
         a0 += part[(long long)r * 2 * H + c];
         a1 += part[(long long)(r + stride) * 2 * H + c];
@@ -1329,14 +1330,14 @@
         a3 += part[(long long)(r + 3 * stride) * 2 * H + c];
     }
     for (; r < rows; r += stride) a0 += part[(long long)r * 2 * H + c];
-    atomicAdd(c < H ? dgamma + c : dbeta + (c - H), (a0 + a1) + (a2 + a3));
+    atomicAdd(c < H ? A.dgamma[l] + c : A.dbeta[l] + (c - H), (a0 + a1) + (a2 + a3));
 }
 
 template <typename T>
 __global__ __launch_bounds__(256) void stack_input_norm_kernel(
     const T* __restrict__ x, const float* __restrict__ gamma, const float* __restrict__ beta,
-    bf16_t* __restrict__ out, float* __restrict__ mean_out, float* __restrict__ rstd_out, int B,
-    int Tn, int D, float eps) {
+    bf16_t* __restrict__ out, bf16_t* __restrict__ xhat, float* __restrict__ mean_out,
+    float* __restrict__ rstd_out, int B, int Tn, int D, float eps) {
     const int lane = threadIdx.x & 63, wave = threadIdx.x >> 6;
     const long long rows = (long long)B * Tn;
     for (long long row = (long long)blockIdx.x * 4 + wave; row < rows; row += (long long)gridDim.x * 4) {
@@ -1358,30 +1359,68 @@
         bf16_t* o = out + ((long long)t * B + b) * D;
         for (int c = lane; c < D; c += 64)
             o[c] = f32_to_bf16((ElemIO<T>::load(xr + c) - m) * rs * gamma[c] + beta[c]);
-    }
-}
-
-template <typename T>
-__global__ __launch_bounds__(256) void stack_input_norm_bwd_kernel(
-    const T* __restrict__ x, const bf16_t* __restrict__ dX, const float* __restrict__ mean_in,
-    const float* __restrict__ rstd_in, float* __restrict__ dgamma, float* __restrict__ dbeta, int B,
-    int Tn, int D, int rows_per_block) {
-    const int c = threadIdx.x;
-    if (c >= D) return;
-    const long long rows = (long long)B * Tn;
-    const long long r0 = (long long)blockIdx.x * rows_per_block;
-    const long long r1 = min(rows, r0 + rows_per_block);
-    float ag = 0.f, ab = 0.f;
-    for (long long row = r0; row < r1; ++row) {
-        const int t = (int)(row / B), b = (int)(row % B);
-        const long long xrow = (long long)b * Tn + t;
-        const float dy = bf16_to_f32(dX[row * D + c]);
-        const float xh = (ElemIO<T>::load(x + xrow * D + c) - mean_in[xrow]) * rstd_in[xrow];
-        ag += dy * xh;
-        ab += dy;
-    }
-    atomicAdd(dgamma + c, ag);
-    atomicAdd(dbeta + c, ab);
+        if (xhat) {
+            bf16_t* h = xhat + ((long long)t * B + b) * (D + 8);
+            for (int c = lane; c < D; c += 64) h[c] = f32_to_bf16((ElemIO<T>::load(xr + c) - m) * rs);
+            if (lane < 8) h[D + lane] = f32_to_bf16(lane == 0 ? 1.f : 0.f);
+        }
+    }
+}
+
+constexpr int ING_ROWS = 16;
+__global__ __launch_bounds__(256) void stack_input_norm_grad_kernel(
+    const float* __restrict__ P, long long slice_stride, int S, const bf16_t* __restrict__ W, int D,
+    float* __restrict__ part) {
+    extern __shared__ float ing_red[];
+    const int lane = threadIdx.x & 63, wave = threadIdx.x >> 6;
+    const int ldp = D + 8;
+    const int k0 = blockIdx.x * ING_ROWS + wave * 4;
+    float c[4];
+#pragma unroll
+    for (int rr = 0; rr < 4; ++rr) {
+        const float* p = P + (long long)(k0 + rr) * ldp + D;
+        float a = 0.f;
+        for (int sl = 0; sl < S; ++sl) a += p[sl * slice_stride];
+        c[rr] = a;
+    }
+    for (int j = lane * 4; j < D; j += 256) {
+        float ag[4] = {0.f, 0.f, 0.f, 0.f}, ab[4] = {0.f, 0.f, 0.f, 0.f};
+#pragma unroll
+        for (int rr = 0; rr < 4; ++rr) {
+            const float* p = P + (long long)(k0 + rr) * ldp + j;
+            float4 v = make_float4(0.f, 0.f, 0.f, 0.f);
+            for (int sl = 0; sl < S; ++sl) {
+                const float4 u = *reinterpret_cast<const float4*>(p + sl * slice_stride);
+                v.x += u.x; v.y += u.y; v.z += u.z; v.w += u.w;
+            }
+            const uint2 wv = *reinterpret_cast<const uint2*>(W + (long long)(k0 + rr) * D + j);
+            const float w0 = bf16_to_f32((bf16_t)(wv.x & 0xffffu)), w1 = bf16_to_f32((bf16_t)(wv.x >> 16));
+            const float w2 = bf16_to_f32((bf16_t)(wv.y & 0xffffu)), w3 = bf16_to_f32((bf16_t)(wv.y >> 16));
+            ag[0] += w0 * v.x; ag[1] += w1 * v.y; ag[2] += w2 * v.z; ag[3] += w3 * v.w;
+            ab[0] += w0 * c[rr]; ab[1] += w1 * c[rr]; ab[2] += w2 * c[rr]; ab[3] += w3 * c[rr];
+        }
+        float* rg = ing_red + (long long)wave * 2 * D + j;
+        *reinterpret_cast<float4*>(rg) = make_float4(ag[0], ag[1], ag[2], ag[3]);
+        *reinterpret_cast<float4*>(rg + D) = make_float4(ab[0], ab[1], ab[2], ab[3]);
+    }
+    __syncthreads();
+    float* out = part + (long long)blockIdx.x * 2 * D;
+    for (int i = threadIdx.x; i < 2 * D; i += 256)
+        out[i] = ((ing_red[i] + ing_red[2 * D + i]) + ing_red[4 * D + i]) + ing_red[6 * D + i];
+}
+__global__ __launch_bounds__(256) void stack_input_norm_grad_sum_kernel(const float* __restrict__ part, int rows, int D,
+                                                                        float* __restrict__ dgamma,
+                                                                        float* __restrict__ dbeta) {
+    __shared__ float red[4][64];
+    const int i = blockIdx.x * 64 + (threadIdx.x & 63), q = threadIdx.x >> 6;
+    float a = 0.f;
+    if (i < 2 * D)
+        for (int r = q; r < rows; r += 4) a += part[(long long)r * 2 * D + i];
+    red[q][threadIdx.x & 63] = a;
+    __syncthreads();
+    if (q != 0 || i >= 2 * D) return;
+    float* dst = i < D ? dgamma : dbeta;
+    if (dst) dst[i < D ? i : i - D] += (red[0][threadIdx.x] + red[1][threadIdx.x]) + (red[2][threadIdx.x] + red[3][threadIdx.x]);
 }
 
 __global__ void stack_init_state_kernel(const float* __restrict__ h0, const float* __restrict__ c0,
@@ -1537,45 +1576,44 @@
     return ED_OK;
 }
 
-int ed_stack_sum_parts(const float* part, int rows, int H, float* dgamma, float* dbeta, hipStream_t s) {
-    if (rows <= 0) return ED_OK;
-    const int gy = rows >= 64 ? 16 : 1;
-    hipLaunchKernelGGL(stack_sum_parts_kernel, dim3((2 * H + 255) / 256, gy), dim3(256), 0, s, part,
-                       rows, H, dgamma, dbeta);
+int ed_stack_sum_parts(EdSumParts A, hipStream_t s) {
+    if (A.n <= 0) return ED_OK;
+    int gy = 1;
+    for (int l = 0; l < A.n; ++l) {
+        A.gy[l] = A.rows[l] >= 64 ? 16 : 1;
+        gy = max(gy, A.gy[l]);
+    }
+    hipLaunchKernelGGL(stack_sum_parts_kernel, dim3((2 * A.H + 255) / 256, gy, A.n), dim3(256), 0, s, A);
     ED_CHECK_LAUNCH("stack_sum_parts_kernel");
     return ED_OK;
 }
 
 int ed_stack_input_norm(int x_dtype, const void* x, const float* gamma, const float* beta,
-                        bf16_t* out, float* mean, float* rstd, int B, int T, int D, float eps,
+                        bf16_t* out, bf16_t* xhat, float* mean, float* rstd, int B, int T, int D, float eps,
                         hipStream_t s) {
     const int grid = ed_grid_for((long long)B * T, 4, 256 * 16);
     if (x_dtype == ED_F32)
         hipLaunchKernelGGL(stack_input_norm_kernel<float>, dim3(grid), dim3(256), 0, s,
-                           (const float*)x, gamma, beta, out, mean, rstd, B, T, D, eps);
+                           (const float*)x, gamma, beta, out, xhat, mean, rstd, B, T, D, eps);
     else
         hipLaunchKernelGGL(stack_input_norm_kernel<bf16_t>, dim3(grid), dim3(256), 0, s,
-                           (const bf16_t*)x, gamma, beta, out, mean, rstd, B, T, D, eps);
+                           (const bf16_t*)x, gamma, beta, out, xhat, mean, rstd, B, T, D, eps);
     ED_CHECK_LAUNCH("stack_input_norm_kernel");
     return ED_OK;
 }
 
-int ed_stack_input_norm_bwd(int x_dtype, const void* x, const bf16_t* dX, const float* mean,
-                            const float* rstd, float* dgamma, float* dbeta, int B, int T, int D,
-                            hipStream_t s) {
-    const long long rows = (long long)B * T;
-    const int rpb = 64;
-    const int grid = (int)((rows + rpb - 1) / rpb);
-    const int threads = (D + 63) / 64 * 64;
-    if (x_dtype == ED_F32)
-        hipLaunchKernelGGL(stack_input_norm_bwd_kernel<float>, dim3(grid), dim3(threads), 0, s,
-                           (const float*)x, dX, mean, rstd, dgamma, dbeta, B, T, D, rpb);
-    else
-        hipLaunchKernelGGL(stack_input_norm_bwd_kernel<bf16_t>, dim3(grid), dim3(threads), 0, s,
-                           (const bf16_t*)x, dX, mean, rstd, dgamma, dbeta, B, T, D, rpb);
-    ED_CHECK_LAUNCH("stack_input_norm_bwd_kernel");
+int ed_stack_input_norm_grad(const float* partials, long long slice_stride, int slices, const bf16_t* wih_p, int H,
+                             int D, float* part, float* dgamma, float* dbeta, hipStream_t s) {
+    const int rows = 4 * H / ING_ROWS;
+    hipLaunchKernelGGL(stack_input_norm_grad_kernel, dim3(rows), dim3(256), (size_t)8 * D * sizeof(float), s, partials,
+                       slice_stride, slices, wih_p, D, part);
+    ED_CHECK_LAUNCH("stack_input_norm_grad_kernel");
+    hipLaunchKernelGGL(stack_input_norm_grad_sum_kernel, dim3((2 * D + 63) / 64), dim3(256), 0, s, part, rows, D, dgamma,
+                       dbeta);
+    ED_CHECK_LAUNCH("stack_input_norm_grad_sum_kernel");
     return ED_OK;
 }
+size_t ed_stack_input_norm_grad_part_bytes(int H, int D) { return (size_t)(4 * H / ING_ROWS) * 2 * D * sizeof(float); }
 
 int ed_stack_init_state(const float* h0, const float* c0, bf16_t* Yx0, float* Cx0, bf16_t* hfrag,
                         int B, int H, hipStream_t s) {
diff --git a/edgedict_amd/csrc/stack_kernels.hpp b/edgedict_amd/csrc/stack_kernels.hpp
--- a/edgedict_amd/csrc/stack_kernels.hpp
+++ b/edgedict_amd/csrc/stack_kernels.hpp
@@ -146,13 +146,21 @@
                     bf16_t* dz, float* part, int grid, int B, int H, int t0, int t1, int reduce,
                     hipStream_t s, unsigned drop_thresh = 0, unsigned drop_seed = 0, float drop_scale = 1.f,
                     int drop_T = 0);
-int ed_stack_sum_parts(const float* part, int rows, int H, float* dgamma, float* dbeta, hipStream_t s);
+struct EdSumParts {
+    int n, H;
+    const float* part[ED_STACK_MAX_SLOTS];
+    int rows[ED_STACK_MAX_SLOTS];
+    int gy[ED_STACK_MAX_SLOTS];
+    float* dgamma[ED_STACK_MAX_SLOTS];
+    float* dbeta[ED_STACK_MAX_SLOTS];
+};
+int ed_stack_sum_parts(EdSumParts A, hipStream_t s);
 int ed_stack_input_norm(int x_dtype, const void* x, const float* gamma, const float* beta,
-                        bf16_t* out, float* mean, float* rstd, int B, int T, int D, float eps,
+                        bf16_t* out, bf16_t* xhat, float* mean, float* rstd, int B, int T, int D, float eps,
                         hipStream_t s);
-int ed_stack_input_norm_bwd(int x_dtype, const void* x, const bf16_t* dX, const float* mean,
-                            const float* rstd, float* dgamma, float* dbeta, int B, int T, int D,
-                            hipStream_t s);
+int ed_stack_input_norm_grad(const float* partials, long long slice_stride, int slices, const bf16_t* wih_p, int H,
+                             int D, float* part, float* dgamma, float* dbeta, hipStream_t s);
+size_t ed_stack_input_norm_grad_part_bytes(int H, int D);
 struct EdInitStates {
     int n, B, H;
     const float* h0[8];
diff --git a/edgedict_amd/encoder_stack.py b/edgedict_amd/encoder_stack.py
--- a/edgedict_amd/encoder_stack.py
+++ b/edgedict_amd/encoder_stack.py
@@ -42,6 +42,7 @@
 DW_AT_END = 2
 ACCUM_GRADS = 8
 INFERENCE = 64
+INPUT_NORM_FROZEN = 128
 
 CHUNK = int(os.environ.get("EDGEDICT_STACK_CHUNK", "16"))
 LAG = int(os.environ.get("EDGEDICT_STACK_LAG", "0"))
@@ -269,8 +270,10 @@
             dig, dib = in_norm[0].grad, in_norm[1].grad
             d.flags |= ACCUM_GRADS
         else:
-            dig = zeros[2 * H * self.L:2 * H * self.L + self.I0]
-            dib = zeros[2 * H * self.L + self.I0:]
+            dig = dib = None
+            if not d.flags & INPUT_NORM_FROZEN:
+                dig = zeros[2 * H * self.L:2 * H * self.L + self.I0]
+                dib = zeros[2 * H * self.L + self.I0:]
             d.flags &= ~ACCUM_GRADS
         dout = dout.contiguous()
         d.dout, d.d_in_gamma, d.d_in_beta = _p(dout), _p(dig), _p(dib)
@@ -312,8 +315,11 @@
         if x.dtype not in (F32, BF16):
             x = x.float()
         needs_bwd = any(ctx.needs_input_grad)
+        mode = 0 if needs_bwd else INFERENCE
+        if needs_bwd and not any(ctx.needs_input_grad[1:3]):
+            mode = INPUT_NORM_FROZEN
         plan = _Plan(x, (in_g, in_b), layers, list(reductions), h0, c0,
-                     (FLAGS if flags is None else flags) | (0 if needs_bwd else INFERENCE), drop)
+                     (FLAGS if flags is None else flags) | mode, drop)
         with ops.timed("enc_stack_fwd_T%d_L%d" % (x.shape[1], len(layers))):
             plan.forward()
         hN, cN = plan.final_states()
diff --git a/include/edgedict_hip.h b/include/edgedict_hip.h
--- a/include/edgedict_hip.h
+++ b/include/edgedict_hip.h
@@ -246,6 +246,7 @@
 #define EDGEDICT_STACK_DW_AT_END 2
 #define EDGEDICT_STACK_ACCUM_GRADS 8
 #define EDGEDICT_STACK_INFERENCE 64
+#define EDGEDICT_STACK_INPUT_NORM_FROZEN 128
 #define EDGEDICT_STACK_SIDE_STREAM_PER_LAYER 4
 
 typedef struct edgedict_stack_desc {
```

New measurement: 3377 utterances/s. Within noise of the previous version (-0.0%).
